# wenxuanliu/multimodal-vae

Measured on AMD Instinct MI355X. Metric: ELBO-steps/sec (whole node), MultiMNIST b=256 per GPU, higher is better.
Workload: dtype bf16; 1 GPU; multimnist_50x50_conv_mmvae_gru_text_3pass_elbo_step; batch_per_gpu=256, global_batch=256, n_latents=100, parallelism=dp1, hip_graph=False, optimizer=adam, mfma=bf16 in / fp32 acc; fp32 master weights, BN stats, PoE/KL/BCE/NLL, Adam

## Files before the change

### multimodal-vae_amd/csrc/convres.hip

```cpp
#include "gemm.h"
#include "convres_geo.h"
#include "convres.h"
#include "bn_dev.h"
#include "convres_epi.h"
#include <type_traits>
#include <cstdlib>

namespace {


template <int I, int N, typename F>
__device__ __forceinline__ void static_for(F&& f) {
    if constexpr (I < N) {
        f(std::integral_constant<int, I>{});
        static_for<I + 1, N>(f);
    }
}

struct ConvResArgs {
    const bf16* A;
    int nimg, group_n;
    const bf16* Wp[4];
    int Kpad[4];
    int Npad;
    bf16* out;
    int ldo;
    float2* colstats;
    const bf16* d_r;
    const float2* d_affine;
    const float2* d_meanrstd;
    float2* d_red;
    int dbg;
    BnFinalizeArgs fin;
    const bf16* t_r;
    const float2* t_red;
    const float2* t_mr;
    const float* t_gamma;
    float* t_dgamma; float* t_dbeta;
    float t_inv_cnt;
    int t_groups;
    bf16* stage_out;
    unsigned long long* ts;
};

constexpr unsigned OOB_OFF = 0x40000000u;

template <class G, int NI>
constexpr int tab_base(int c) {
    int r = 0;
    for (int i = 0; i < c; ++i) r += crgeo::cdiv(NI * G::OYX(i), 32) * 32;
    return r;
}

template <class G, int NI, int CH, int WAVES, int NG, bool SCR_OWN, int NSPLIT = 1, int KSPL = 1>
struct CrLayout {
    static constexpr int NTHR = WAVES * 64;
    static constexpr int MG = WAVES / (NG * KSPL), NT = G::N / 32 / NSPLIT / NG;
    static constexpr int max_mt() { int m = 0; for (int c = 0; c < G::NCLS; ++c) m = crgeo::cmax(m, crgeo::cdiv(crgeo::cdiv(NI * G::OYX(c), 32), MG)); return m; }
    static constexpr int RED_BYTES = KSPL > 1 ? WAVES * max_mt() * NT * 4096 : 0;
    static constexpr bool BDIR = CH == 0;
    static constexpr int BP = (CH * 16 + 8) * 2;
    static constexpr int W_BYTES = BDIR ? 0 : G::N * BP;
    static_assert(!BDIR || SCR_OWN, "direct-B kernels have no weight buffer to lend to the epilogue");
    static constexpr int IMG_ALL = NI * G::IMG_BYTES;
    static constexpr int TAB_BYTES = tab_base<G, NI>(G::NCLS) * 4;
    static constexpr int SCR_PITCH = 80, SCR_BYTES = 32 * SCR_PITCH;
    static constexpr int TRT_BYTES = G::C * 16;
    static constexpr int OFF_W = IMG_ALL, OFF_TAB = OFF_W + W_BYTES, OFF_TRT = OFF_TAB + TAB_BYTES,
                         OFF_SCR = OFF_TRT + TRT_BYTES, OFF_RED = OFF_SCR + (SCR_OWN ? WAVES * SCR_BYTES : 0), TOTAL = OFF_RED + RED_BYTES;
    static_assert((NSPLIT == 1 && KSPL == 1) || BDIR, "column / k splits exist for the direct-B kernels only");
    static_assert(G::N % (32 * NSPLIT * NG) == 0 && WAVES % (NG * KSPL) == 0, "wave decomposition");
    static_assert(SCR_OWN || W_BYTES >= WAVES * SCR_BYTES, "the weight buffer doubles as the epilogue scratch");
    static_assert(TOTAL <= 160 * 1024, "LDS budget");
};

template <class G, int NI, int CH, int WAVES, int NG, bool SCR_OWN, int MODE, int TR, int NSPLIT = 1, int KSPL = 1>
__global__ __launch_bounds__(WAVES * 64) void convres_kernel(const ConvResArgs a) {
    using L = CrLayout<G, NI, CH, WAVES, NG, SCR_OWN, NSPLIT, KSPL>;
    constexpr int NT = L::NT, MG = L::MG, NTHR = WAVES * 64;
    constexpr int BP = L::BP, SCR_PITCH = L::SCR_PITCH;
    extern __shared__ __attribute__((aligned(16))) char smem[];
    char* const img_s = smem;
    char* const w_s = smem + L::OFF_W;
    unsigned* const tab = reinterpret_cast<unsigned*>(smem + L::OFF_TAB);
    float4* const trt = reinterpret_cast<float4*>(smem + L::OFF_TRT);

    const int tid = threadIdx.x, lane = tid & 63;
    const int wave = __builtin_amdgcn_readfirstlane(tid >> 6);
    const int r = lane & 31, h = lane >> 5;
    const int kg = wave % KSPL, ng = (wave / KSPL) % NG, mg = wave / (KSPL * NG);
    const int ntb = blockIdx.y * (G::N / 32 / NSPLIT) + ng * NT;
    const int img0 = blockIdx.x * NI;
    const int grp = img0 / a.group_n;
    auto stamp = [&](int idx) {
        if (a.ts && lane == 0) a.ts[((size_t)blockIdx.x * WAVES + wave) * 16 + idx] = __builtin_amdgcn_s_memrealtime();
    };
    stamp(0);

    constexpr bool BDIR = L::BDIR;
    constexpr int WV = BDIR ? 1 : crgeo::cdiv(G::N * CH * 2, NTHR);
    i32x4c wreg[WV];
    auto w_fetch = [&](auto ci, auto chi) {
        constexpr int c = decltype(ci)::value, ch = decltype(chi)::value;
        constexpr int CHK = crgeo::cmin(CH, G::KSTEPS(c) - ch * CH), VPR = CHK * 2 + (BDIR ? 1 : 0), NV = G::N * VPR;
        const bf16* wsrc = a.Wp[c] + ch * CH * 16;
        const int kpad = a.Kpad[c];
#pragma unroll
        for (int it = 0; it < crgeo::cdiv(NV, NTHR); ++it) {
            const int v = tid + it * NTHR;
            const int n = v / VPR, kv = v - n * VPR;
            if (v < NV) wreg[it] = *reinterpret_cast<const i32x4c*>(wsrc + (size_t)n * kpad + kv * 8);
        }
    };
    auto w_store = [&](auto ci, auto chi) {
        constexpr int c = decltype(ci)::value, ch = decltype(chi)::value;
        constexpr int CHK = crgeo::cmin(CH, G::KSTEPS(c) - ch * CH), VPR = CHK * 2 + (BDIR ? 1 : 0), NV = G::N * VPR;
#pragma unroll
        for (int it = 0; it < crgeo::cdiv(NV, NTHR); ++it) {
            const int v = tid + it * NTHR;
            const int n = v / VPR, kv = v - n * VPR;
            if (v < NV) *reinterpret_cast<i32x4c*>(w_s + n * BP + kv * 16) = wreg[it];
        }
    };
    if constexpr (!BDIR) w_fetch(std::integral_constant<int, 0>{}, std::integral_constant<int, 0>{});

    constexpr int VPP = G::C / 8;
    constexpr int NVI = NI * G::AH * G::AW * VPP;
    constexpr int IT = crgeo::cdiv(NVI, NTHR), SB = 4, NB = crgeo::cdiv(IT, SB);
    static_assert(NTHR % VPP == 0, "a thread keeps its channel vector across staging iterations");
    const bf16* const src = a.A + (size_t)img0 * (G::AH * G::AW * G::C);
    const bf16* const src_r = TR == 2 ? a.t_r + (size_t)img0 * (G::AH * G::AW * G::C) : nullptr;
    bf16* const stage_dst = (TR != 0 && a.stage_out && blockIdx.y == 0) ? a.stage_out + (size_t)img0 * (G::AH * G::AW * G::C) : nullptr;
    i32x4c ireg[SB], rreg[TR == 2 ? SB : 1];
    auto i_fetch = [&](int b) {
#pragma unroll
        for (int i = 0; i < SB; ++i) {
            const int v = tid + (b * SB + i) * NTHR;
            if (b * SB + i < IT && v < NVI) {
                ireg[i] = *reinterpret_cast<const i32x4c*>(src + (size_t)v * 8);
                if constexpr (TR == 2) rreg[i] = *reinterpret_cast<const i32x4c*>(src_r + (size_t)v * 8);
            }
        }
    };
    float tc0[TR ? 8 : 1], tc1[TR ? 8 : 1], tc2[TR == 2 ? 8 : 1];
    auto i_store = [&](int b) {
#pragma unroll
        for (int i = 0; i < SB; ++i) {
            const int v = tid + (b * SB + i) * NTHR;
            if (b * SB + i < IT && v < NVI) {
                const int pix = v / VPP, cv = v - pix * VPP;
                const int img = pix / (G::AH * G::AW), p2 = pix - img * (G::AH * G::AW);
                const int iy = p2 / G::AW, ix = p2 - iy * G::AW;
                const int cell = G::cell(iy, ix);
                i32x4c val = ireg[i];
                if constexpr (TR == 1) {
                    const bf16x8 x = __builtin_bit_cast(bf16x8, val);
                    bf16x8 o;
#pragma unroll
                    for (int j = 0; j < 8; ++j) o[j] = (bf16)swish_fast((float)x[j] * tc0[j] + tc1[j]);
                    val = __builtin_bit_cast(i32x4c, o);
                } else if constexpr (TR == 2) {
                    const bf16x8 x = __builtin_bit_cast(bf16x8, val), rr = __builtin_bit_cast(bf16x8, rreg[i]);
                    bf16x8 o;
#pragma unroll
                    for (int j = 0; j < 8; ++j) o[j] = (bf16)((float)x[j] * tc0[j] + ((float)rr[j] * tc1[j] + tc2[j]));
                    val = __builtin_bit_cast(i32x4c, o);
                }
                if (cell >= 0) *reinterpret_cast<i32x4c*>(img_s + img * G::IMG_BYTES + cell + cv * 16) = val;
                if constexpr (TR != 0)
                    if (stage_dst) *reinterpret_cast<i32x4c*>(stage_dst + (size_t)v * 8) = val;
            }
        }
    };
    if (!(a.dbg & 4)) i_fetch(0);

    {
        const i32x4c z = {0, 0, 0, 0};
        for (int i = tid * 16; i < L::IMG_ALL; i += NTHR * 16) *reinterpret_cast<i32x4c*>(img_s + i) = z;
        const unsigned img_out = (unsigned)(G::OH * G::OW) * (unsigned)a.ldo * 2u;
        static_for<0, G::NCLS>([&](auto ci) {
            constexpr int c = decltype(ci)::value;
            constexpr int ROWS = NI * G::OYX(c), T = crgeo::cdiv(ROWS, 32);
            for (int e = tid; e < T * 32; e += NTHR) {
                unsigned v = OOB_OFF;
                if (e < ROWS) {
                    const int img = e / G::OYX(c), q = e - img * G::OYX(c);
                    const int jy = q / G::OX(c), jx = q - jy * G::OX(c);
                    v = (unsigned)img * img_out + (unsigned)((G::out_y(c, jy) * G::OW + G::out_x(c, jx)) * a.ldo * 2);
                }
                tab[tab_base<G, NI>(c) + e] = v;
            }
        });
        if constexpr (TR == 1) {
            for (int ch = tid; ch < G::C; ch += NTHR) {
                float2 aff, mr;
                bn_channel_tables(a.fin, grp, ch, aff, mr);
                trt[ch] = make_float4(aff.x, aff.y, 0.f, 0.f);
            }
            if (blockIdx.x == 0 && blockIdx.y == 0) {
                for (int i = tid; i < a.fin.G * G::C; i += NTHR) {
                    float2 aff, mr;
                    bn_channel_tables(a.fin, i / G::C, i % G::C, aff, mr);
                    a.fin.affine[i] = aff; a.fin.meanrstd[i] = mr;
                }
                bn_running_update(a.fin, tid, NTHR);
            }
        } else if constexpr (TR == 2) {
            for (int ch = tid; ch < G::C; ch += NTHR) {
                float sx = 0.f, sy = 0.f;
                for (int q = 0; q < MMVAE_STAT_SLOTS; ++q) {
                    const float2 t = a.t_red[((size_t)grp * MMVAE_STAT_SLOTS + q) * G::C + ch];
                    sx += t.x; sy += t.y;
                }
                const float2 mr = a.t_mr[grp * G::C + ch];
                const float g = a.t_gamma[ch] * mr.y, m1 = sx * a.t_inv_cnt, m2 = sy * a.t_inv_cnt;
                const float cb = -g * m2 * mr.y;
                trt[ch] = make_float4(g, cb, -cb * mr.x - g * m1, 0.f);
            }
            if (blockIdx.x == 0 && blockIdx.y == 0 && (a.t_dgamma || a.t_dbeta)) {
                for (int ch = tid; ch < G::C; ch += NTHR) {
                    float tg = 0.f, tb = 0.f;
                    for (int gg = 0; gg < a.t_groups; ++gg)
                        for (int q = 0; q < MMVAE_STAT_SLOTS; ++q) {
                            const float2 t = a.t_red[((size_t)gg * MMVAE_STAT_SLOTS + q) * G::C + ch];
                            tb += t.x; tg += t.y;
                        }
                    if (a.t_dgamma) a.t_dgamma[ch] += tg;
                    if (a.t_dbeta) a.t_dbeta[ch] += tb;
                }
            }
        }
    }
    stamp(1);
    __syncthreads();
    stamp(2);
    if constexpr (TR != 0) {
        const int cv0 = (tid % VPP) * 8;
#pragma unroll
        for (int j = 0; j < 8; ++j) {
            const float4 t = trt[cv0 + j];
            tc0[j] = t.x; tc1[j] = t.y;
            if constexpr (TR == 2) tc2[j] = t.z;
        }
    }
    if (!(a.dbg & 4)) {
        i_store(0);
        for (int b = 1; b < NB; ++b) { i_fetch(b); i_store(b); }
    }
    if constexpr (!BDIR) w_store(std::integral_constant<int, 0>{}, std::integral_constant<int, 0>{});
    stamp(3);
    __syncthreads();
    stamp(4);

    const __amdgpu_buffer_rsrc_t orsrc = __builtin_amdgcn_make_buffer_rsrc(
        a.out, 0, (int)((size_t)a.nimg * G::OH * G::OW * a.ldo * 2), 0x00020000);
    const __amdgpu_buffer_rsrc_t rrsrc = __builtin_amdgcn_make_buffer_rsrc(
        const_cast<bf16*>(a.d_r ? a.d_r : a.out), 0, (int)((size_t)a.nimg * G::OH * G::OW * a.ldo * 2), 0x00020000);
    const unsigned wg_out = (unsigned)img0 * (unsigned)(G::OH * G::OW) * (unsigned)a.ldo * 2u;
    float dsc[NT], dsh[NT], dmean[NT], drstd[NT], s1[NT], s2[NT];
#pragma unroll
    for (int nt = 0; nt < NT; ++nt) {
        const int co = (ntb + nt) * 32 + r;
        dsc[nt] = 1.f; dsh[nt] = 0.f; dmean[nt] = 0.f; drstd[nt] = 0.f; s1[nt] = 0.f; s2[nt] = 0.f;
        if (MODE == 1 && a.d_affine) { const float2 t = a.d_affine[grp * G::N + co]; dsc[nt] = t.x; dsh[nt] = t.y; }
        if (MODE == 1 && a.d_meanrstd) { const float2 t = a.d_meanrstd[grp * G::N + co]; dmean[nt] = t.x; drstd[nt] = t.y; }
    }
    char* const scr = (SCR_OWN ? smem + L::OFF_SCR : w_s) + wave * L::SCR_BYTES;
    __amdgpu_buffer_rsrc_t wrsrc[BDIR ? G::NCLS : 1];
    if constexpr (BDIR) {
#pragma unroll
        for (int i = 0; i < G::NCLS; ++i)
            wrsrc[i] = __builtin_amdgcn_make_buffer_rsrc(const_cast<bf16*>(a.Wp[i]), 0, a.Npad * a.Kpad[i] * 2, 0x00020000);
    }

    static_for<0, G::NCLS>([&](auto ci) {
        constexpr int c = decltype(ci)::value;
        constexpr int ROWS = NI * G::OYX(c), T = crgeo::cdiv(ROWS, 32), MT = crgeo::cdiv(T, MG);
        constexpr int KS = G::KSTEPS(c), CHE = BDIR ? KS : CH, NCH = crgeo::cdiv(KS, CHE);
        constexpr int KSL = KS / KSPL;
        int abase[MT];
#pragma unroll
        for (int m = 0; m < MT; ++m) {
            const int t = mg + m * MG;
            int R = (t < T ? t : 0) * 32 + r;
            R = R < ROWS ? R : ROWS - 1;
            const int img = R / G::OYX(c), q = R - img * G::OYX(c);
            const int jy = q / G::OX(c), jx = q - jy * G::OX(c);
            abase[m] = img * G::IMG_BYTES + G::base0(c) + jy * G::row_stride(c) + jx * G::col_stride(c) + h * 16;
            if constexpr (KSPL > 1) {
                static_assert(G::TH(c) % KSPL == 0, "the k split is by tap row");
                constexpr int KSL_ = KS / KSPL;
                abase[m] += kg * (G::step_off(c, KSL_) - G::step_off(c, 0));
            }
        }
        f32x16 acc[MT][NT];
#pragma unroll
        for (int m = 0; m < MT; ++m)
#pragma unroll
            for (int nt = 0; nt < NT; ++nt)
#pragma unroll
                for (int j = 0; j < 16; ++j) acc[m][nt][j] = 0.f;
        const int wrow = ((ng * NT) * 32 + r) * BP + h * 16;

        if constexpr (BDIR) {
            constexpr int PD = KSL < 8 ? KSL : 8;
            static_assert(KSPL == 1 || KSL % 2 == 0, "a wave's k range starts on a 32-column block of the packed weights");
            unsigned voff[NT];
#pragma unroll
            for (int nt = 0; nt < NT; ++nt)
                voff[nt] = (unsigned)(((2 * (ntb + nt) + (r >> 4)) * (a.Kpad[c] >> 5) * 64 + h * 16 + (r & 15)) * 16) +
                           (unsigned)(kg * (KSL / 2) * 1024);
            auto bload = [&](auto ki, bf16x8 (&fb)[NT]) {
                constexpr int kk = decltype(ki)::value;
#pragma unroll
                for (int nt = 0; nt < NT; ++nt)
                    fb[nt] = __builtin_bit_cast(bf16x8, __builtin_amdgcn_raw_buffer_load_b128(wrsrc[c], (int)voff[nt], (kk >> 1) * 1024 + (kk & 1) * 512, 0));
            };
            auto aload = [&](auto ki, bf16x8 (&fa)[MT]) {
                constexpr int kk = decltype(ki)::value;
                constexpr int aoff = G::step_off(c, kk);
#pragma unroll
                for (int m = 0; m < MT; ++m) fa[m] = *reinterpret_cast<const bf16x8*>(img_s + abase[m] + aoff);
            };
            bf16x8 bq[PD][NT], af[MT];
            static_for<0, PD>([&](auto pi) { bload(pi, bq[decltype(pi)::value]); });
            aload(std::integral_constant<int, 0>{}, af);
            __builtin_amdgcn_sched_group_barrier(0x100, MT, 0);
            if (!(a.dbg & 2))
            static_for<0, KSL>([&](auto ki) {
                constexpr int kk = decltype(ki)::value;
                constexpr int KS = KSL;
                bf16x8 bcur[NT], an[MT];
#pragma unroll
                for (int nt = 0; nt < NT; ++nt) bcur[nt] = bq[kk % PD][nt];
                if constexpr (kk + PD < KS) bload(std::integral_constant<int, kk + PD>{}, bq[kk % PD]);
                if constexpr (kk + 1 < KS) aload(std::integral_constant<int, kk + 1>{}, an);
#pragma unroll
                for (int m = 0; m < MT; ++m)
#pragma unroll
                    for (int nt = 0; nt < NT; ++nt)
                        acc[m][nt] = __builtin_amdgcn_mfma_f32_32x32x16_bf16(af[m], bcur[nt], acc[m][nt], 0, 0, 0);
                if constexpr (kk + PD < KS) __builtin_amdgcn_sched_group_barrier(0x020, NT, 0);
                if constexpr (kk + 1 < KS) __builtin_amdgcn_sched_group_barrier(0x100, MT, 0);
                __builtin_amdgcn_sched_group_barrier(0x008, MT * NT, 0);
                if constexpr (kk + 1 < KS) {
#pragma unroll
                    for (int m = 0; m < MT; ++m) af[m] = an[m];
                }
            });
            if constexpr (KSPL > 1) {
                float* const red = reinterpret_cast<float*>(smem + L::OFF_RED);
                constexpr int WSTR = L::max_mt() * NT * 1024;
#pragma unroll
                for (int m = 0; m < MT; ++m)
#pragma unroll
                    for (int nt = 0; nt < NT; ++nt)
#pragma unroll
                        for (int v4 = 0; v4 < 4; ++v4)
                            *reinterpret_cast<f32x4*>(red + wave * WSTR + ((m * NT + nt) * 64 + lane) * 16 + v4 * 4) =
                                f32x4{acc[m][nt][4 * v4], acc[m][nt][4 * v4 + 1], acc[m][nt][4 * v4 + 2], acc[m][nt][4 * v4 + 3]};
                __syncthreads();
                if (kg == 0) {
#pragma unroll
                    for (int k2 = 1; k2 < KSPL; ++k2)
#pragma unroll
                        for (int m = 0; m < MT; ++m)
#pragma unroll
                            for (int nt = 0; nt < NT; ++nt)
#pragma unroll
                                for (int v4 = 0; v4 < 4; ++v4) {
                                    const f32x4 t = *reinterpret_cast<const f32x4*>(red + (wave + k2) * WSTR + ((m * NT + nt) * 64 + lane) * 16 + v4 * 4);
                                    acc[m][nt][4 * v4] += t[0]; acc[m][nt][4 * v4 + 1] += t[1];
                                    acc[m][nt][4 * v4 + 2] += t[2]; acc[m][nt][4 * v4 + 3] += t[3];
                                }
                }
                __syncthreads();
            }
        }
        static_for<0, NCH>([&](auto chi) {
            constexpr int ch = decltype(chi)::value;
            constexpr int CHK = crgeo::cmin(CHE, KS - ch * CHE);
            constexpr bool last_chunk = ch + 1 == NCH;
            constexpr bool has_next = !BDIR && (!last_chunk || c + 1 < G::NCLS);
            constexpr int cn = last_chunk ? c + 1 : c, chn = last_chunk ? 0 : ch + 1;
            if constexpr (has_next) w_fetch(std::integral_constant<int, cn>{}, std::integral_constant<int, chn>{});
            if (!BDIR && !(a.dbg & 2)) {
                bf16x8 af[MT], bfr[NT];
                auto frag = [&](auto ki, bf16x8 (&fa)[MT], bf16x8 (&fb)[NT]) {
                    constexpr int kk = decltype(ki)::value;
                    constexpr int aoff = G::step_off(c, ch * CHE + kk);
#pragma unroll
                    for (int nt = 0; nt < NT; ++nt)
                        fb[nt] = *reinterpret_cast<const bf16x8*>(w_s + wrow + nt * 32 * BP + kk * 32);
#pragma unroll
                    for (int m = 0; m < MT; ++m) fa[m] = *reinterpret_cast<const bf16x8*>(img_s + abase[m] + aoff);
                };
                frag(std::integral_constant<int, 0>{}, af, bfr);
                __builtin_amdgcn_sched_group_barrier(0x100, MT + NT, 0);
                static_for<0, CHK>([&](auto ki) {
                    constexpr int kk = decltype(ki)::value;
                    bf16x8 an[MT], bn[NT];
                    if constexpr (kk + 1 < CHK) frag(std::integral_constant<int, kk + 1>{}, an, bn);
#pragma unroll
                    for (int m = 0; m < MT; ++m)
#pragma unroll
                        for (int nt = 0; nt < NT; ++nt)
                            acc[m][nt] = __builtin_amdgcn_mfma_f32_32x32x16_bf16(af[m], bfr[nt], acc[m][nt], 0, 0, 0);
                    if constexpr (kk + 1 < CHK) __builtin_amdgcn_sched_group_barrier(0x100, MT + NT, 0);
                    __builtin_amdgcn_sched_group_barrier(0x008, MT * NT, 0);
                    if constexpr (kk + 1 < CHK) {
#pragma unroll
                        for (int m = 0; m < MT; ++m) af[m] = an[m];
#pragma unroll
                        for (int nt = 0; nt < NT; ++nt) bfr[nt] = bn[nt];
                    }
                });
            }
            if constexpr (last_chunk) {
                stamp(5 + 2 * c);
                if constexpr (!SCR_OWN) __syncthreads();
#pragma unroll
                for (int m = 0; m < MT; ++m) {
                    const int t = mg + m * MG;
                    if (t < T && kg == 0) {
                        const unsigned* trow = tab + tab_base<G, NI>(c) + t * 32;
                        const unsigned off0 = trow[lane & 15], off1 = trow[16 + (lane & 15)];
                        const int rows_left = ROWS - t * 32;
#pragma unroll
                        for (int nt = 0; nt < NT; ++nt) {
                            const unsigned cob = (unsigned)(((ntb + nt) * 32 + (lane >> 4) * 8) * 2) + wg_out;
                            if (rows_left >= 32)
                                cr_epilogue_tile<MODE, false>(acc[m][nt], scr, lane, 32, off0 + cob, off1 + cob, orsrc, rrsrc,
                                                              dsc[nt], dsh[nt], dmean[nt], drstd[nt], s1[nt], s2[nt], !(a.dbg & 1));
                            else
                                cr_epilogue_tile<MODE, true>(acc[m][nt], scr, lane, rows_left, off0 + cob, off1 + cob, orsrc, rrsrc,
                                                             dsc[nt], dsh[nt], dmean[nt], drstd[nt], s1[nt], s2[nt], !(a.dbg & 1));
                        }
                    }
                }
            }
            if constexpr (last_chunk) stamp(6 + 2 * c);
            if constexpr (has_next) {
                __syncthreads();
                w_store(std::integral_constant<int, cn>{}, std::integral_constant<int, chn>{});
                __syncthreads();
            }
        });
    });

    stamp(13);
    float2* red = MODE == 1 ? a.d_red : a.colstats;
    if (red && kg == 0) {
        const int slot = (int)(blockIdx.x + wave) % MMVAE_STAT_SLOTS;
#pragma unroll
        for (int nt = 0; nt < NT; ++nt) {
            const float t1 = s1[nt] + __shfl_xor(s1[nt], 32, 64), t2 = s2[nt] + __shfl_xor(s2[nt], 32, 64);
            if (h == 0) {
                float2* d = red + ((size_t)grp * MMVAE_STAT_SLOTS + slot) * G::N + (ntb + nt) * 32 + r;
                atomicAdd(&d->x, t1);
                atomicAdd(&d->y, t2);
            }
        }
    }
    stamp(14);
}

}

namespace {

template <class G>
bool geo_matches(const GemmParams& p) {
    const GatherCommon& c = p.c;
    if (c.C != G::C || c.Ald != G::C || c.N != G::N || c.AH != G::AH || c.AW != G::AW || c.OH != G::OH || c.OW != G::OW) return false;
    if (c.nclasses != G::NCLS) return false;
    if (G::FORM == 0) {
        if (c.sy != G::S || c.sx != G::S || c.dy != 1 || c.dx != 1 || c.osy != 1 || c.osx != 1) return false;
    } else {
        if (c.sy != 1 || c.sx != 1 || c.dy != -1 || c.dx != -1 || c.osy != G::S || c.osx != G::S) return false;
    }
    for (int i = 0; i < G::NCLS; ++i) {
        const GatherClass& k = p.cls[i];
        if (k.OY != G::OY(i) || k.OX != G::OX(i) || k.TH != G::TH(i) || k.TW != G::TW(i) || k.offy != G::offy(i) ||
            k.offx != G::offx(i) || k.ooy != G::ph(i) || k.oox != G::pw(i) || k.K != G::K(i) || k.Kpad < G::K(i))
            return false;
    }
    return true;
}

template <class G, int NI, int CH, int WAVES, int NG, bool SCR_OWN, int MODE, int TR, int NSPLIT, int KSPL>
int launch_cr_mode(const ConvResArgs& a, hipStream_t stream) {
    using L = CrLayout<G, NI, CH, WAVES, NG, SCR_OWN, NSPLIT, KSPL>;
    static std::atomic<unsigned> attr_set{0};
    if (mmvae_first_use_on_device(attr_set))
        hipFuncSetAttribute(reinterpret_cast<const void*>(&convres_kernel<G, NI, CH, WAVES, NG, SCR_OWN, MODE, TR, NSPLIT, KSPL>),
                            hipFuncAttributeMaxDynamicSharedMemorySize, 160 * 1024);
    MMVAE_LAUNCH((convres_kernel<G, NI, CH, WAVES, NG, SCR_OWN, MODE, TR, NSPLIT, KSPL>), dim3(a.nimg / NI, NSPLIT), dim3(WAVES * 64), L::TOTAL, stream, a);
    MMVAE_TRY(mmvae_check_launch("convres"));
    return 1;
}

template <class G, int NI, int CH, int WAVES, int NG, bool SCR_OWN, int NSPLIT = 1, int KSPL = 1>
int launch_cr(const GemmParams& p, hipStream_t stream) {
    const GatherCommon& c = p.c;
    const int nimg = c.groups * c.group_n;
    ConvResArgs a{};
    a.A = c.A; a.nimg = nimg; a.group_n = c.group_n;
    constexpr bool BDIR = CH == 0;
    for (int i = 0; i < G::NCLS; ++i) {
        a.Wp[i] = BDIR ? p.cls[i].Wf : p.cls[i].Wp; a.Kpad[i] = p.cls[i].Kpad;
        if (BDIR && (!a.Wp[i] || a.Kpad[i] % 32 != 0)) return 0;
    }
    a.Npad = p.npad;
    a.out = p.out_bf; a.ldo = p.ldo; a.colstats = p.colstats;
    a.dbg = mmvae_knob("convres_dbg", 0);
    a.ts = reinterpret_cast<unsigned long long*>(((unsigned long long)(unsigned)mmvae_knob("convres_ts_hi", 0) << 32) |
                                                 (unsigned)mmvae_knob("convres_ts_lo", 0));
    a.d_r = p.d_r; a.d_affine = p.d_affine; a.d_meanrstd = p.d_meanrstd; a.d_red = p.d_red;
    const int kind = p.tr ? p.tr->kind : 0;
    MMVAE_REQUIRE(!(p.tr && p.tr->out == c.A) || NSPLIT == 1, "convres: an in-place staging by-product needs one workgroup per image tile");
    if (mmvae_probe_on()) {
        char tag[96];
        snprintf(tag, sizeof(tag), "convres form%d %d>%d %dx%d>%dx%d k%d s%d %s tr%d img%d", G::FORM, G::C, G::N, G::AH, G::AW, G::OH, G::OW,
                 G::KH, G::S, p.d_r ? "dgrad" : "fwd", kind, nimg);
        mmvae_probe_tag(tag, 2.0 * (G::FORM == 0 ? G::OH * G::OW : G::AH * G::AW) * G::KH * G::KW * G::C * G::N * (double)nimg);
    }
    if (kind == 1) {
        a.fin = p.tr->fin; a.stage_out = p.tr->out;
        MMVAE_REQUIRE(a.fin.C == G::C && a.fin.G == c.groups && a.fin.affine && a.fin.meanrstd && a.fin.gamma && a.fin.beta,
                      "convres: BatchNorm tables of the staged operand do not match the layer");
        MMVAE_REQUIRE(!p.d_r, "convres: forward-type staging transform on a data-gradient launch");
        return launch_cr_mode<G, NI, CH, WAVES, NG, SCR_OWN, 0, 1, NSPLIT, KSPL>(a, stream);
    }
    if (kind == 2) {
        const GatherTransform& t = *p.tr;
        MMVAE_REQUIRE(p.d_r && t.r && t.red && t.mr && t.gamma && t.groups == c.groups, "convres: BatchNorm-backward staging needs r / sums / tables");
        a.t_r = t.r; a.t_red = t.red; a.t_mr = t.mr; a.t_gamma = t.gamma; a.t_dgamma = t.dgamma; a.t_dbeta = t.dbeta;
        a.t_inv_cnt = t.inv_cnt; a.t_groups = t.groups; a.stage_out = t.out;
        return launch_cr_mode<G, NI, CH, WAVES, NG, SCR_OWN, 1, 2, NSPLIT, KSPL>(a, stream);
    }
    return p.d_r ? launch_cr_mode<G, NI, CH, WAVES, NG, SCR_OWN, 1, 0, NSPLIT, KSPL>(a, stream)
                 : launch_cr_mode<G, NI, CH, WAVES, NG, SCR_OWN, 0, 0, NSPLIT, KSPL>(a, stream);
}

bool features_ok(const GemmParams& p) {
    const GatherCommon& c = p.c;
    if (!p.out_bf || p.out_f || p.out_act_bf || p.e_mask || p.d_mask || p.d_colsum || p.d_cmod > 0 || p.d_bcast_n > 0) return false;
    if (c.a_bcast_n > 0 || c.a_mask || c.a_affine || c.a_act != ACT_NONE) return false;
    if (p.ldo != c.N || p.bias) return false;
    if (p.d_r && (p.d_ld != p.ldo || p.d_act != ACT_SWISH)) return false;
    if (p.colstats && p.d_r) return false;
    if ((size_t)c.groups * c.group_n * c.OH * c.OW * p.ldo * 2 >= (size_t)OOB_OFF) return false;
    return true;
}

template <class G, int NI, int CH, int WAVES, int NG, bool SCR_OWN, int NSPLIT = 1, int KSPL = 1>
int try_cr(const GemmParams& p, hipStream_t stream) {
    if (!geo_matches<G>(p)) return 0;
    if (p.c.group_n % NI != 0) return 0;
    return launch_cr<G, NI, CH, WAVES, NG, SCR_OWN, NSPLIT, KSPL>(p, stream);
}

using crgeo::Geo;
typedef Geo<0, 32, 64, 25, 25, 12, 12, 4, 4, 2, 1> G_mm_conv2;
typedef Geo<0, 64, 128, 12, 12, 6, 6, 4, 4, 2, 1> G_mm_conv3;
typedef Geo<1, 128, 64, 6, 6, 12, 12, 4, 4, 2, 1> G_mm_convT2;
typedef Geo<1, 64, 32, 12, 12, 25, 25, 5, 5, 2, 1> G_mm_convT3;
typedef Geo<1, 64, 32, 12, 12, 25, 25, 4, 4, 2, 1> G_mm_conv2d;
typedef Geo<0, 32, 64, 25, 25, 12, 12, 5, 5, 2, 1> G_mm_convT3d;
typedef Geo<1, 256, 128, 2, 2, 6, 6, 4, 4, 2, 0> G_mm_convT1;
typedef Geo<0, 128, 256, 6, 6, 2, 2, 4, 4, 2, 0> G_mm_conv4;
typedef Geo<0, 32, 64, 32, 32, 16, 16, 4, 4, 2, 1> G_ca_conv2;
typedef Geo<0, 64, 128, 16, 16, 8, 8, 4, 4, 2, 1> G_ca_conv3;
typedef Geo<1, 128, 64, 8, 8, 16, 16, 4, 4, 2, 1> G_ca_convT2;
typedef Geo<1, 64, 32, 16, 16, 32, 32, 4, 4, 2, 1> G_ca_convT3;

}

int try_launch_convres(const GemmParams& p, hipStream_t stream) {
    const bool forced = p.tr && p.tr->kind != 0;
    if ((!mmvae_knob("convres", 1) && !forced) || !features_ok(p)) {
        MMVAE_REQUIRE(!forced, "convres: a staging transform was requested for a launch this path does not cover");
        return 0;
    }
    int rc;
    const int nimg = p.c.groups * p.c.group_n;
    const int alt = mmvae_knob("convres_alt", 0);
    if ((rc = try_cr<G_mm_conv2, 1, 16, 8, 2, true>(p, stream)) != 0) return rc;
    if (alt != 3) {
        if ((rc = try_cr<G_mm_conv3, 2, 0, 8, 4, true>(p, stream)) != 0) return rc;
        if (nimg <= 256) { if ((rc = try_cr<G_mm_convT2, 2, 0, 8, 2, true>(p, stream)) != 0) return rc; }
        if ((rc = try_cr<G_mm_convT2, 4, 0, 8, 2, true>(p, stream)) != 0) return rc;
    }
    if ((rc = try_cr<G_mm_conv3, 2, 8, 8, 4, true>(p, stream)) != 0) return rc;
    if (nimg <= 256) { if ((rc = try_cr<G_mm_convT2, 2, 8, 4, 1, true>(p, stream)) != 0) return rc; }
    if ((rc = try_cr<G_mm_convT2, 4, 16, 8, 2, true>(p, stream)) != 0) return rc;
    if (alt == 1) { if ((rc = try_cr<G_mm_convT3, 4, 20, 8, 1, false>(p, stream)) != 0) return rc; }
    if ((rc = try_cr<G_mm_convT3, 2, 16, 4, 1, false>(p, stream)) != 0) return rc;
    if ((rc = try_cr<G_mm_conv2d, 1, 16, 8, 1, true>(p, stream)) != 0) return rc;
    if (alt != 4) {
        if (nimg > 256 && alt != 5) { if ((rc = try_cr<G_mm_convT1, 16, 0, 5, 1, true, 4, 1>(p, stream)) != 0) return rc; }
        if ((rc = try_cr<G_mm_convT1, 8, 0, 6, 1, true, 4, 2>(p, stream)) != 0) return rc;
        if ((rc = try_cr<G_mm_conv4, 8, 0, 8, 2, true, 4, 4>(p, stream)) != 0) return rc;
    }
    if ((rc = try_cr<G_mm_convT3d, 2, 10, 8, 2, false>(p, stream)) != 0) return rc;
    if (mmvae_knob("convres_celeba", 1)) {
        if ((rc = try_cr<G_ca_conv2, 1, 16, 8, 2, true>(p, stream)) != 0) return rc;
        if ((rc = try_cr<G_ca_conv3, 2, 0, 8, 4, true>(p, stream)) != 0) return rc;
        if ((rc = try_cr<G_ca_convT2, 4, 0, 8, 2, true>(p, stream)) != 0) return rc;
        if ((rc = try_cr<G_ca_convT3, 2, 16, 4, 1, false>(p, stream)) != 0) return rc;
    }
    MMVAE_REQUIRE(!forced, "convres: no kernel is compiled for the geometry of a launch with a staging transform");
    return 0;
}
```

### multimodal-vae_amd/csrc/convres_geo.h

```cpp
#pragma once

namespace crgeo {

constexpr int cdiv(int a, int b) { return (a + b - 1) / b; }
constexpr int fdiv(int a, int b) { return a >= 0 ? a / b : -((-a + b - 1) / b); }
constexpr int cmax(int a, int b) { return a > b ? a : b; }
constexpr int cmin(int a, int b) { return a < b ? a : b; }

template <int FORM_, int C_, int N_, int AH_, int AW_, int OH_, int OW_, int KH_, int KW_, int S_, int PAD_, int PIXPAD_ = 16>
struct Geo {
    static constexpr int FORM = FORM_, C = C_, N = N_, AH = AH_, AW = AW_, OH = OH_, OW = OW_, KH = KH_, KW = KW_, S = S_, PAD = PAD_;
    static constexpr int NCLS = FORM == 0 ? 1 : S * S;
    static constexpr int PIX = C * 2 + PIXPAD_;
    static constexpr int KSTEP_PER_TAP = C / 16;
    static_assert(C % 8 == 0 && N % 32 == 0, "channel counts");

    static constexpr int ph(int c) { return FORM == 0 ? 0 : c / S; }
    static constexpr int pw(int c) { return FORM == 0 ? 0 : c % S; }
    static constexpr int kh0(int c) { return (ph(c) + PAD) % S; }
    static constexpr int kw0(int c) { return (pw(c) + PAD) % S; }
    static constexpr int OY(int c) { return FORM == 0 ? OH : (OH - ph(c) + S - 1) / S; }
    static constexpr int OX(int c) { return FORM == 0 ? OW : (OW - pw(c) + S - 1) / S; }
    static constexpr int TH(int c) { return FORM == 0 ? KH : (KH - kh0(c) + S - 1) / S; }
    static constexpr int TW(int c) { return FORM == 0 ? KW : (KW - kw0(c) + S - 1) / S; }
    static constexpr int offy(int c) { return FORM == 0 ? -PAD : (ph(c) + PAD - kh0(c)) / S; }
    static constexpr int offx(int c) { return FORM == 0 ? -PAD : (pw(c) + PAD - kw0(c)) / S; }
    static constexpr int K(int c) { return TH(c) * TW(c) * C; }
    static constexpr int KSTEPS(int c) { return K(c) / 16; }
    static constexpr int OYX(int c) { return OY(c) * OX(c); }
    static constexpr int TPI(int c) { return cdiv(OYX(c), 32); }
    static constexpr int osy() { return FORM == 0 ? 1 : S; }
    static constexpr int out_y(int c, int jy) { return jy * osy() + ph(c); }
    static constexpr int out_x(int c, int jx) { return jx * osy() + pw(c); }
    static constexpr int gy(int c, int jy, int ty) { return FORM == 0 ? jy * S - PAD + ty : jy + offy(c) - ty; }
    static constexpr int gx(int c, int jx, int tx) { return FORM == 0 ? jx * S - PAD + tx : jx + offx(c) - tx; }

    static constexpr int DMIN = fdiv(-PAD, S), DMAX = fdiv(KW - 1 - PAD, S);
    static constexpr int PW0 = OW + DMAX - DMIN;
    static constexpr int LR0 = (OH - 1) * S + KH;
    static constexpr int ring_lo(bool x) {
        int r = 0;
        for (int c = 0; c < NCLS; ++c) r = cmax(r, x ? TW(c) - 1 - offx(c) : TH(c) - 1 - offy(c));
        return r;
    }
    static constexpr int ring_hi(bool x) {
        int r = 0;
        for (int c = 0; c < NCLS; ++c) r = cmax(r, x ? OX(c) - 1 + offx(c) - (AW - 1) : OY(c) - 1 + offy(c) - (AH - 1));
        return r;
    }
    static constexpr int RT = FORM == 1 ? ring_lo(false) : 0, RB = FORM == 1 ? ring_hi(false) : 0;
    static constexpr int RL = FORM == 1 ? ring_lo(true) : 0, RR = FORM == 1 ? ring_hi(true) : 0;
    static constexpr int AHP = RT + AH + RB, AWP = RL + AW + RR;
    static constexpr int IMG_BYTES = FORM == 0 ? LR0 * S * PW0 * PIX : AHP * AWP * PIX;

    static constexpr int cell(int iy, int ix) {
        if (FORM == 0) {
            const int row = iy + PAD, plane = ix % S, col = ix / S - DMIN;
            if (row < 0 || row >= LR0 || col < 0 || col >= PW0) return -1;
            return ((row * S + plane) * PW0 + col) * PIX;
        }
        return ((iy + RT) * AWP + ix + RL) * PIX;
    }
    static constexpr int row_stride(int) { return FORM == 0 ? S * S * PW0 * PIX : AWP * PIX; }
    static constexpr int col_stride(int) { return PIX; }
    static constexpr int base0(int c) {
        return FORM == 0 ? 0 : ((offy(c) + RT - (TH(c) - 1)) * AWP + offx(c) + RL - (TW(c) - 1)) * PIX;
    }
    static constexpr int tap_off(int c, int ty, int tx) {
        if (FORM == 0) {
            const int e = tx - PAD, d = fdiv(e, S), p = e - d * S;
            return ((ty * S + p) * PW0 + d - DMIN) * PIX;
        }
        return ((TH(c) - 1 - ty) * AWP + (TW(c) - 1 - tx)) * PIX;
    }
    static constexpr int step_tap(int kk) { return kk / KSTEP_PER_TAP; }
    static constexpr int step_c0(int kk) { return (kk % KSTEP_PER_TAP) * 16; }
    static constexpr int step_off(int c, int kk) {
        const int tap = step_tap(kk);
        return tap_off(c, tap / TW(c), tap % TW(c)) + step_c0(kk) * 2;
    }
    static constexpr int max_ksteps() { int r = 0; for (int c = 0; c < NCLS; ++c) r = cmax(r, KSTEPS(c)); return r; }
    static constexpr int max_tpi() { int r = 0; for (int c = 0; c < NCLS; ++c) r = cmax(r, TPI(c)); return r; }
    static constexpr int tab_entries() { int r = 0; for (int c = 0; c < NCLS; ++c) r += TPI(c) * 32; return r; }
    static constexpr int tab_base(int c) { int r = 0; for (int i = 0; i < c; ++i) r += TPI(i) * 32; return r; }
};

}
```

### multimodal-vae_amd/csrc/gemm.h

```cpp
#pragma once
#include "common.h"
#include "elementwise.h"
#include <vector>

#define MMVAE_MAX_CLASSES 4

struct GatherClass {
    int OY, OX;
    int rows_per_group;
    int TH, TW;
    int offy, offx;
    int ooy, oox;
    int K;
    int Kpad;
    const bf16* Wp;
    const bf16* Wf;
    float* dWp;
};

struct GatherCommon {
    int groups, group_n;
    const bf16* A;
    int AH, AW, Ald, C;
    int sy, sx, dy, dx;
    const float2* a_affine;
    int a_act;
    const uint8_t* a_mask;
    float a_mask_scale;
    int a_bcast_n;
    int OH, OW, osy, osx;
    int N;
    int nclasses;
};

struct GatherTransform {
    int kind;
    BnFinalizeArgs fin;
    const bf16* r;
    const float2* red;
    const float2* mr;
    const float* gamma;
    float* dgamma; float* dbeta;
    float inv_cnt;
    int groups;
    bf16* out;
};

struct GemmParams {
    GatherCommon c;
    GatherClass cls[MMVAE_MAX_CLASSES];
    int ksplit;
    float* sk_buf;
    unsigned* sk_cnt;
    const float* bias;
    bf16* out_bf;
    float* out_f;
    int ldo;
    bf16* out_act_bf;
    int e_act;
    const uint8_t* e_mask;
    float e_mask_scale;
    float2* colstats;
    const bf16* d_r;
    int d_ld;
    int d_bcast_n;
    const float2* d_affine;
    int d_act;
    const uint8_t* d_mask;
    float d_mask_scale;
    const float2* d_meanrstd;
    float2* d_red;
    float* d_colsum;
    int npad;
    const GatherTransform* tr;
    int d_cmod;
};

struct WgradParams {
    GatherCommon c;
    GatherClass cls[MMVAE_MAX_CLASSES];
    const bf16* P;
    int ldp;
    const float2* p_affine;
    int p_act;
    int rows_per_block;
    float* slab;
    long long slab_chunk_stride;
    long long slab_cls_off[MMVAE_MAX_CLASSES];
};

struct WgradSlabJob { float* dst; const float* slab; int N, K, Kpad, chunks; long long chunk_stride; hipStream_t stream;
                      int src_ld; };
struct WgradRingJob { float* dst; const float* slab; int N, Kpad, C, Kc, copies, ntx, ty0, tx0, st, kw; hipStream_t stream; };
struct WgradSlabCtx {
    float* pool = nullptr;
    size_t cap = 0, used = 0;
    std::vector<WgradSlabJob> jobs;
    std::vector<WgradRingJob> ring_jobs;
    void reset(float* p, size_t c) { pool = p; cap = c; used = 0; jobs.clear(); ring_jobs.clear(); }
    float* take(size_t n) {
        n = (n + 3) / 4 * 4;
        if (!pool || used + n > cap) return nullptr;
        float* p = pool + used;
        used += n;
        return p;
    }
};

int launch_gemm_gather(const GemmParams& p, hipStream_t stream);
int try_launch_gemm_small(const GemmParams& p, hipStream_t stream);
int launch_wgrad(const WgradParams& p, hipStream_t stream, WgradSlabCtx* ctx = nullptr);
int launch_wgrad_group(const WgradParams* list, int n, hipStream_t stream, WgradSlabCtx* ctx = nullptr);
int launch_wgrad_reduce(WgradSlabCtx* ctx, hipStream_t stream, bool only_own = false);
```

### multimodal-vae_amd/csrc/multimnist.hip

```cpp
#include "multimnist.h"
#include <memory>
#include "mlp_tail.h"
#include "plan_base.h"
#include "thin.h"
#include <cstring>

namespace {
constexpr int IMG = 50, NPIX = 2500;
}

struct MMPlan : PlanBase {
    int ldz, kx, kz;
    ConvL conv[4], convT[4];
    LinL fc[3], up;
    BnL bn[6];
    struct GruIdx { int wih, whh, wihT, whhT, g_wih, g_whh; long long bih, bhh; } te_f, te_r, td0, td1;
    const float* step_image = nullptr;
    hipEvent_t ev_dz = nullptr;
    hipEvent_t ev_txtgrads = nullptr;
    int te_h2p, te_h2pT, g_te_h2p, td_z2h, td_z2hT, g_td_z2h, td_h2o, td_h2oT, g_td_h2o;
    bool mlp_tail = false;
    int mt_w2, mt_w3, mt_w3t, mt_w2t;
    struct W {
        char* zero_begin; size_t zero_bytes;
        float2 *st_e[3], *red_e[3], *st_d[3], *red_d[3];
        float* sums; float* dz_img; float* dz_txt;
        float2 *aff_e[3], *mr_e[3], *aff_d[3], *mr_d[3];
        bf16 *patches1, *r1, *r2, *r3, *r4, *y1, *y2;
        bf16 *a1, *a2, *a3, *a4, *ay1, *ay2, *au, *aq1, *aq2, *aq3;
        float* encout; uint8_t *m1, *m2, *gkeep;
        float *txtout, *te_gates_f, *te_gates_r; bf16 *te_x, *te_hprev, *te_hsum;
        float *eps, *mu, *logvar, *z_f32; bf16* z_bf;
        bf16 *u, *q1, *q2, *q3; float *logits, *recon, *dlogit;
        float *words, *dwords, *td_gates; long long* tokens;
        bf16 *td_x0, *td_h0p, *td_mid, *td_h1p, *td_hz, *td_zbf;
        bf16 *dgi0, *dgh0, *dgi1, *dgh1, *dlogit_bf, *dhinit;
        bf16 *patches4, *d3, *d2, *d1, *du;
        bf16 *d_encout; float* d_txtout; bf16* te_dout_bf; bf16 *te_dgi_f, *te_dgh_f, *te_dgi_r;
        bf16 *dy2, *dy1, *db4, *dr4, *d3e, *d2e, *d1e;
        bf16 *d3r, *d2r, *d1r, *d3er, *d2er;
        float* tmp_f32;
        float* slab; size_t slab_floats;
    } w;
};

namespace {

void build_params(MMPlan& P) {
    const int D = P.D;
    auto bn = [&](const std::string& n, int c) { add_param(P, n + ".weight", {c}); add_param(P, n + ".bias", {c}); };
    auto gru = [&](const std::string& n, int inp, const char* sfx) {
        add_param(P, n + ".weight_ih_" + sfx, {300, inp}); add_param(P, n + ".weight_hh_" + sfx, {300, 100});
        add_param(P, n + ".bias_ih_" + sfx, {300}); add_param(P, n + ".bias_hh_" + sfx, {300});
    };
    add_param(P, "image_encoder.features.0.weight", {32, 1, 4, 4});
    add_param(P, "image_encoder.features.2.weight", {64, 32, 4, 4}); bn("image_encoder.features.3", 64);
    add_param(P, "image_encoder.features.5.weight", {128, 64, 4, 4}); bn("image_encoder.features.6", 128);
    add_param(P, "image_encoder.features.8.weight", {256, 128, 4, 4}); bn("image_encoder.features.9", 256);
    add_param(P, "image_encoder.classifier.0.weight", {400, 1024}); add_param(P, "image_encoder.classifier.0.bias", {400});
    add_param(P, "image_encoder.classifier.3.weight", {200, 400}); add_param(P, "image_encoder.classifier.3.bias", {200});
    add_param(P, "image_encoder.classifier.6.weight", {2 * D, 200}); add_param(P, "image_encoder.classifier.6.bias", {2 * D});
    add_param(P, "image_decoder.upsample.0.weight", {1024, D}); add_param(P, "image_decoder.upsample.0.bias", {1024});
    add_param(P, "image_decoder.hallucinate.0.weight", {256, 128, 4, 4}); bn("image_decoder.hallucinate.1", 128);
    add_param(P, "image_decoder.hallucinate.3.weight", {128, 64, 4, 4}); bn("image_decoder.hallucinate.4", 64);
    add_param(P, "image_decoder.hallucinate.6.weight", {64, 32, 5, 5}); bn("image_decoder.hallucinate.7", 32);
    add_param(P, "image_decoder.hallucinate.9.weight", {32, 1, 4, 4});
    add_param(P, "text_encoder.embed.weight", {12, 100});
    gru("text_encoder.gru", 100, "l0"); gru("text_encoder.gru", 100, "l0_reverse");
    add_param(P, "text_encoder.h2p.weight", {2 * D, 100}); add_param(P, "text_encoder.h2p.bias", {2 * D});
    add_param(P, "text_decoder.embed.weight", {12, 100});
    add_param(P, "text_decoder.z2h.weight", {100, D}); add_param(P, "text_decoder.z2h.bias", {100});
    gru("text_decoder.gru", 100 + D, "l0"); gru("text_decoder.gru", 100, "l1");
    add_param(P, "text_decoder.h2o.weight", {12, 100 + D}); add_param(P, "text_decoder.h2o.bias", {12});
}

void build_plan(MMPlan& P) {
    const int D = P.D;
    P.ldz = round_up(D + 1, 8); P.kz = round_up(D, 32); P.kx = round_up(100 + D, 32);
    build_params(P);
    const char* bnn[6] = {"image_encoder.features.3", "image_encoder.features.6", "image_encoder.features.9",
                          "image_decoder.hallucinate.1", "image_decoder.hallucinate.4", "image_decoder.hallucinate.7"};
    const int bnc[6] = {64, 128, 256, 128, 64, 32};
    long long so = 0;
    for (int i = 0; i < 6; ++i) {
        P.bn[i] = BnL{off(P, std::string(bnn[i]) + ".weight"), off(P, std::string(bnn[i]) + ".bias"), bnc[i], so, i};
        P.bn_names.push_back(bnn[i]); P.bn_list.push_back(P.bn[i]);
        so += 2 * bnc[i];
    }
    build_conv(P, P.conv[0], "image_encoder.features.0.weight", ConvGeom{1, 32, 4, 4, 2, 1, 50, 50, 25, 25, false}, -1, false, true, false);
    build_conv(P, P.conv[1], "image_encoder.features.2.weight", ConvGeom{32, 64, 4, 4, 2, 1, 25, 25, 12, 12, false}, 0, true, false, false);
    build_conv(P, P.conv[2], "image_encoder.features.5.weight", ConvGeom{64, 128, 4, 4, 2, 1, 12, 12, 6, 6, false}, 1, true, false, false);
    build_conv(P, P.conv[3], "image_encoder.features.8.weight", ConvGeom{128, 256, 4, 4, 2, 0, 6, 6, 2, 2, false}, 2, true, false, false);
    build_conv(P, P.convT[0], "image_decoder.hallucinate.0.weight", ConvGeom{256, 128, 4, 4, 2, 0, 2, 2, 6, 6, true}, 3, true, false, false);
    build_conv(P, P.convT[1], "image_decoder.hallucinate.3.weight", ConvGeom{128, 64, 4, 4, 2, 1, 6, 6, 12, 12, true}, 4, true, false, false);
    build_conv(P, P.convT[2], "image_decoder.hallucinate.6.weight", ConvGeom{64, 32, 5, 5, 2, 1, 12, 12, 25, 25, true}, 5, true, false, false);
    build_conv(P, P.convT[3], "image_decoder.hallucinate.9.weight", ConvGeom{32, 1, 4, 4, 2, 1, 25, 25, 50, 50, true}, -1, true, false, true);
    add_frag_packs(P, P.conv[2]);
    add_frag_packs(P, P.convT[1]);
    add_frag_packs(P, P.conv[3]);
    add_frag_packs(P, P.convT[0]);

    {
        LinL& f = P.fc[0];
        f.w_off = off(P, "image_encoder.classifier.0.weight"); f.b_off = off(P, "image_encoder.classifier.0.bias");
        f.N = 400; f.K = 1024; f.pk_dgrad = -1;
        PackDesc d = pack_dense(f.w_off, 400, 1024, npad_for(400), 1024, 1024, 0);
        d.TW = 2; d.C = 256; d.s_ty = 2; d.s_tx = 1; d.s_c = 4;
        f.pk_fwd = P.pk.add(d);
        PackDesc gd = d; gd.Npad = round_up(400, 64);
        f.gk = P.gk.add(gd);
        for (int sidx = 0; sidx < 4; ++sidx)
            f.pk_dgrad4[sidx] = P.pk.add(pack_dense(f.w_off + sidx, 256, 400, npad_for(256), round_up(400, 64), 4, 1024));
    }
    auto lin = [&](LinL& f, const std::string& n, int N, int K) {
        f.w_off = off(P, n + ".weight"); f.b_off = off(P, n + ".bias"); f.N = N; f.K = K;
        f.pk_fwd = P.pk.add(pack_dense(f.w_off, N, K, npad_for(N), round_up(round_up(K, 8), 64), K, 1));
        f.gk = P.gk.add(pack_dense(f.w_off, N, K, round_up(N, 64), round_up(round_up(K, 8), 64), K, 1));
        f.pk_dgrad = P.pk.add(pack_dense(f.w_off, K, N, npad_for(K), round_up(round_up(N, 8), 64), 1, K));
    };
    lin(P.fc[1], "image_encoder.classifier.3", 200, 400);
    lin(P.fc[2], "image_encoder.classifier.6", 2 * D, 200);
    if (D == 100) {
        P.mlp_tail = true;
        auto fragd = [&](PackDesc d) { d.frag = 1; return P.pk.add(d); };
        P.mt_w2 = fragd(pack_dense(P.fc[1].w_off, 200, 400, 208, 416, 400, 1));
        P.mt_w3 = fragd(pack_dense(P.fc[2].w_off, 200, 200, 208, 224, 200, 1));
        P.mt_w3t = fragd(pack_dense(P.fc[2].w_off, 200, 200, 208, 224, 1, 200));
        P.mt_w2t = fragd(pack_dense(P.fc[1].w_off, 400, 200, 400, 224, 1, 400));
    }
    {
        LinL& f = P.up;
        f.w_off = off(P, "image_decoder.upsample.0.weight"); f.b_off = off(P, "image_decoder.upsample.0.bias");
        f.N = 1024; f.K = D;
        PackDesc d = pack_dense(f.w_off, 1024, D, npad_for(1024), round_up(P.ldz, 64), 0, 1);
        d.NL = 256; d.s_nhi = D; d.s_nlo = 4 * D;
        d.bias_off = f.b_off; d.b_nhi = 1; d.b_nlo = 4;
        f.pk_fwd = P.pk.add(d);
        PackDesc gd = d; f.gk = P.gk.add(gd);
        PackDesc t = pack_dense(f.w_off, D, 1024, npad_for(D), 1024, 1, 0);
        t.TW = 4; t.C = 256; t.s_ty = 0; t.s_tx = D; t.s_c = 4 * D;
        f.pk_dgrad = P.pk.add(t);
    }
    auto rt = [&](long long w, int N, int K, bool transpose) {
        PackDesc d = transpose ? pack_dense(w, K, N, round_up(K, 16), round_up(N, 32), 1, K) : pack_dense(w, N, K, round_up(N, 16), round_up(K, 32), K, 1);
        d.frag = 1;
        return P.pk.add(d);
    };
    auto gw = [&](long long w, int N, int K, int Kc) {
        return P.gk.add(pack_dense(w, N, K, round_up(N, 64), round_up(Kc, 64), K, 1));
    };
    auto grui = [&](MMPlan::GruIdx& g, const std::string& n, const char* sfx, int inp, int inp_k, bool need_hh) {
        const long long wih = off(P, n + ".weight_ih_" + sfx), whh = off(P, n + ".weight_hh_" + sfx);
        g.bih = off(P, n + ".bias_ih_" + sfx); g.bhh = off(P, n + ".bias_hh_" + sfx);
        g.wih = rt(wih, 300, inp, false); g.wihT = rt(wih, 300, inp, true);
        g.whh = rt(whh, 300, 100, false); g.whhT = rt(whh, 300, 100, true);
        g.g_wih = gw(wih, 300, inp, inp_k);
        g.g_whh = need_hh ? gw(whh, 300, 100, TXT_HP) : -1;
    };
    grui(P.te_f, "text_encoder.gru", "l0", 100, TXT_HP, true);
    grui(P.te_r, "text_encoder.gru", "l0_reverse", 100, TXT_HP, false);
    {
        const long long w = off(P, "text_encoder.h2p.weight");
        P.te_h2p = rt(w, 2 * D, 100, false); P.te_h2pT = rt(w, 2 * D, 100, true); P.g_te_h2p = gw(w, 2 * D, 100, TXT_HP);
    }
    {
        const long long w = off(P, "text_decoder.z2h.weight");
        P.td_z2h = rt(w, 100, D, false); P.td_z2hT = rt(w, 100, D, true); P.g_td_z2h = gw(w, 100, D, P.kz);
    }
    grui(P.td0, "text_decoder.gru", "l0", 100 + D, P.kx, true);
    grui(P.td1, "text_decoder.gru", "l1", 100, TXT_HP, true);
    {
        const long long w = off(P, "text_decoder.h2o.weight");
        P.td_h2o = rt(w, 12, 100 + D, false); P.td_h2oT = rt(w, 12, 100 + D, true); P.g_td_h2o = gw(w, 12, 100 + D, P.kx);
    }
    for (PackDesc& d : P.pk.d) {
        d.part = 0;
        for (const ParamInfo& pi : P.params)
            if (d.src_off >= pi.offset && d.src_off < pi.offset + pi.numel)
                d.part = pi.name.rfind("text_", 0) == 0 ? 1 : pi.name.rfind("image_decoder.", 0) == 0 ? 2 : 0;
    }
    {
        auto late = [&](int idx) { if (idx >= 0) P.pk.d[idx].part = 2; };
        for (int l = 0; l < 4; ++l)
            for (int i = 0; i < 4; ++i) { late(P.conv[l].pk_dgrad[i]); late(P.conv[l].pk_dgrad_f[i]); }
        for (int i = 0; i < 4; ++i) late(P.fc[0].pk_dgrad4[i]);
        late(P.fc[1].pk_dgrad); late(P.fc[2].pk_dgrad);
        if (P.mlp_tail) { late(P.mt_w3t); late(P.mt_w2t); }
    }
    for (PackDesc& d : P.gk.d)
        for (const ParamInfo& pi : P.params)
            if (d.src_off >= pi.offset && d.src_off < pi.offset + pi.numel)
                d.part = pi.name.rfind("image_decoder.", 0) == 0 || pi.name.rfind("text_decoder.", 0) == 0;
}

void carve(MMPlan& P, Workspace& ws) {
    MMPlan::W& w = P.w;
    const size_t B = P.B, D = P.D, B3 = (size_t)P.carve_passes * B, B2 = (size_t)(P.carve_passes < 2 ? P.carve_passes : 2) * B;
    char* z0 = ws.take<char>(0);
    const int ec[3] = {64, 128, 256}, dc[3] = {128, 64, 32};
    const int SS = MMVAE_STAT_SLOTS;
    for (int i = 0; i < 3; ++i) { w.st_e[i] = ws.take<float2>(SS * ec[i]); w.red_e[i] = ws.take<float2>(SS * ec[i]); }
    for (int i = 0; i < 3; ++i) { w.st_d[i] = ws.take<float2>(3 * SS * dc[i]); w.red_d[i] = ws.take<float2>(3 * SS * dc[i]); }
    w.sums = ws.take<float>(16 * MMVAE_LOSS_SLOTS);
    P.sk_cnt = ws.take<unsigned>(1024);
    w.dz_img = ws.take<float>(B3 * D);
    w.dz_txt = ws.take<float>(B3 * D);
    char* z1 = ws.take<char>(0);
    w.zero_begin = z0; w.zero_bytes = (size_t)(z1 - z0);
    for (int i = 0; i < 3; ++i) { w.aff_e[i] = ws.take<float2>(ec[i]); w.mr_e[i] = ws.take<float2>(ec[i]); }
    for (int i = 0; i < 3; ++i) { w.aff_d[i] = ws.take<float2>(3 * dc[i]); w.mr_d[i] = ws.take<float2>(3 * dc[i]); }
    w.patches1 = ws.take<bf16>(B * 625 * 16);
    w.r1 = ws.take<bf16>(B * 625 * 32); w.r2 = ws.take<bf16>(B * 144 * 64); w.r3 = ws.take<bf16>(B * 36 * 128);
    w.r4 = ws.take<bf16>(B * 4 * 256);
    w.y1 = ws.take<bf16>(B2 * 400); w.y2 = ws.take<bf16>(B2 * 200);
    w.a1 = ws.take<bf16>(B * 625 * 32); w.a2 = ws.take<bf16>(B * 144 * 64); w.a3 = ws.take<bf16>(B * 36 * 128);
    w.a4 = ws.take<bf16>(B * 4 * 256); w.ay1 = ws.take<bf16>(B2 * 400); w.ay2 = ws.take<bf16>(B2 * 200);
    w.au = ws.take<bf16>(B3 * 1024); w.aq1 = ws.take<bf16>(B3 * 36 * 128); w.aq2 = ws.take<bf16>(B3 * 144 * 64);
    w.aq3 = ws.take<bf16>(B3 * 625 * 32);
    w.encout = ws.take<float>(B2 * 2 * D);
    w.m1 = ws.take<uint8_t>(B2 * 400); w.m2 = ws.take<uint8_t>(B2 * 200); w.gkeep = ws.take<uint8_t>(4 * B3 * 100);
    w.txtout = ws.take<float>(B * 2 * D);
    w.te_gates_f = ws.take<float>(4 * 5 * B * 100); w.te_gates_r = ws.take<float>(5 * B * 100);
    w.te_x = ws.take<bf16>(4 * B * 128); w.te_hprev = ws.take<bf16>(4 * B * 128); w.te_hsum = ws.take<bf16>(B * 128);
    w.eps = ws.take<float>(B3 * D); w.mu = ws.take<float>(B3 * D); w.logvar = ws.take<float>(B3 * D);
    w.z_f32 = ws.take<float>(B3 * D); w.z_bf = ws.take<bf16>(B3 * P.ldz);
    w.u = ws.take<bf16>(B3 * 1024); w.q1 = ws.take<bf16>(B3 * 36 * 128); w.q2 = ws.take<bf16>(B3 * 144 * 64);
    w.q3 = ws.take<bf16>(B3 * 625 * 32);
    w.logits = ws.take<float>(B3 * NPIX); w.recon = ws.take<float>(B3 * NPIX); w.dlogit = ws.take<float>(B3 * NPIX);
    w.words = ws.take<float>(B3 * 48); w.dwords = ws.take<float>(B3 * 48); w.tokens = ws.take<long long>(B3 * 4);
    w.td_gates = ws.take<float>(4 * 2 * 5 * B3 * 100);
    w.td_x0 = ws.take<bf16>(4 * B3 * P.kx); w.td_hz = ws.take<bf16>(4 * B3 * P.kx);
    w.td_h0p = ws.take<bf16>(4 * B3 * 128); w.td_mid = ws.take<bf16>(4 * B3 * 128); w.td_h1p = ws.take<bf16>(4 * B3 * 128);
    w.td_zbf = ws.take<bf16>(B3 * P.kz);
    w.dgi0 = ws.take<bf16>(4 * B3 * 304); w.dgh0 = ws.take<bf16>(4 * B3 * 304);
    w.dgi1 = ws.take<bf16>(4 * B3 * 304); w.dgh1 = ws.take<bf16>(4 * B3 * 304);
    w.dlogit_bf = ws.take<bf16>(4 * B3 * 16); w.dhinit = ws.take<bf16>(B3 * 112);
    w.patches4 = ws.take<bf16>(B3 * 625 * 16);
    w.d3 = ws.take<bf16>(B3 * 625 * 32); w.d2 = ws.take<bf16>(B3 * 144 * 64); w.d1 = ws.take<bf16>(B3 * 36 * 128);
    w.du = ws.take<bf16>(B3 * 1024);
    w.d_encout = ws.take<bf16>(B2 * 2 * D); w.d_txtout = ws.take<float>(B * 2 * D);
    w.te_dout_bf = ws.take<bf16>(B * round_up(2 * (int)D, 8));
    w.te_dgi_f = ws.take<bf16>(4 * B * 304); w.te_dgh_f = ws.take<bf16>(4 * B * 304); w.te_dgi_r = ws.take<bf16>(B * 304);
    w.dy2 = ws.take<bf16>(B2 * 200); w.dy1 = ws.take<bf16>(B2 * 400);
    w.db4 = ws.take<bf16>(B2 * 1024); w.dr4 = ws.take<bf16>(B * 1024);
    w.d3e = ws.take<bf16>(B * 36 * 128); w.d2e = ws.take<bf16>(B * 144 * 64); w.d1e = ws.take<bf16>(B * 625 * 32);
    w.d3r = ws.take<bf16>(B3 * 625 * 32); w.d2r = ws.take<bf16>(B3 * 144 * 64); w.d1r = ws.take<bf16>(B3 * 36 * 128);
    w.d3er = ws.take<bf16>(B * 36 * 128); w.d2er = ws.take<bf16>(B * 144 * 64);
    w.tmp_f32 = ws.take<float>(B3 * NPIX);
    P.sk_floats = (size_t)256 * 128 * 128;
    P.sk_buf = ws.take<float>(P.sk_floats);
    w.slab_floats = (size_t)(P.carve_passes >= 3 ? 48 : 16) << 20;
    w.slab = ws.take<float>(w.slab_floats);
}

int enc_fwd(MMPlan& P, const float* image, int variants, const uint8_t* m1, const uint8_t* m2, int dropout, int training,
            int bn_updates, float* out, hipStream_t s, bool fuse = false) {
    MMPlan::W& w = P.w;
    const int B = P.B;
    if (fuse && mmvae_knob("mm_conv1_mfma", 1)) {
        const PackDesc& d = P.pk.d[P.conv[0].pk_fwd[0]];
        MMVAE_TRY(launch_conv1_fwd_mfma(image, B, P.buf.packed + d.dst_off, d.Kpad, w.r1, w.a1, s));
    } else {
    MMVAE_TRY(launch_im2col_small(image, B, 1, IMG, IMG, 4, 4, 2, 1, 25, 25, w.patches1, 16, s));
    {
        GatherPlan pl = dense_plan(B * 625, 16, 16, 32);
        GemmParams g = gemm_of(P, pl, P.conv[0].pk_fwd, 1, B * 625);
        g.c.A = w.patches1; g.out_bf = w.r1; g.ldo = 32; g.out_act_bf = w.a1; g.e_act = ACT_SWISH;
        MMVAE_TRY(launch_gemm_gather(g, s));
    }
    }
    bf16* r[4] = {w.r1, w.r2, w.r3, w.r4};
    bf16* a[4] = {w.a1, w.a2, w.a3, w.a4};
    for (int l = 1; l < 4; ++l) {
        const ConvL& L = P.conv[l];
        GemmParams g = gemm_of(P, L.fwd, L.pk_fwd, 1, B, L.pk_fwd_f);
        g.c.A = a[l - 1];
        g.out_bf = r[l]; g.ldo = L.g.Cout;
        g.colstats = training ? w.st_e[l - 1] : nullptr;
        GatherTransform tr{};
        if (fuse && l >= 2) {
            const int prows = B * P.conv[l - 1].g.OH * P.conv[l - 1].g.OW;
            tr.kind = 1;
            tr.fin = bn_fin_args(P, P.bn[P.conv[l - 1].bn], prows, 1, w.st_e[l - 2], bn_updates, w.aff_e[l - 2], w.mr_e[l - 2], training);
            g.c.A = r[l - 1]; g.tr = &tr;
            if (mmvae_knob("mm_stage_out", 1)) tr.out = a[l - 1];
        }
        MMVAE_TRY(launch_gemm_gather(g, s));
        const int rows = B * L.g.OH * L.g.OW;
        if (fuse && l <= 2) continue;
        MMVAE_TRY(bn_act(P, P.bn[L.bn], r[l], a[l], rows, rows, 1, w.st_e[l - 1], bn_updates, w.aff_e[l - 1], w.mr_e[l - 1], training, s));
    }
    const int rows = variants * B;
    const bool drop = training && dropout;
    const float ms = 1.f / (1.f - DROP_P);
    {
        GatherPlan pl = plan_fwdform(2, 2, 1, 1, 256, 2, 2, 1, 0, 400, 1, rows);
        GemmParams g = gemm_of(P, pl, &P.fc[0].pk_fwd, 1, rows);
        g.c.A = w.a4; g.c.a_bcast_n = B;
        g.bias = P.buf.params + P.fc[0].b_off; g.out_bf = w.y1; g.ldo = 400;
        g.out_act_bf = w.ay1; g.e_act = ACT_SWISH; if (drop) { g.e_mask = m1; g.e_mask_scale = ms; }
        MMVAE_TRY(launch_gemm_gather(g, s));
    }
    if (P.mlp_tail) {
        Mlp2FwdArgs a{};
        a.rows = rows; a.x = w.ay1;
        a.w2 = P.buf.packed + P.pk.d[P.mt_w2].dst_off; a.b2 = P.buf.params + P.fc[1].b_off;
        a.w3 = P.buf.packed + P.pk.d[P.mt_w3].dst_off; a.b3 = P.buf.params + P.fc[2].b_off;
        if (drop) { a.mask = m2; a.mask_scale = ms; }
        a.y2 = w.y2; a.ay2 = w.ay2; a.out = out;
        return launch_mlp2_fwd(a, s);
    }
    {
        GatherPlan pl = dense_plan(rows, 400, 400, 200);
        GemmParams g = gemm_of(P, pl, &P.fc[1].pk_fwd, 1, rows);
        g.c.A = w.ay1;
        g.bias = P.buf.params + P.fc[1].b_off; g.out_bf = w.y2; g.ldo = 200;
        g.out_act_bf = w.ay2; g.e_act = ACT_SWISH; if (drop) { g.e_mask = m2; g.e_mask_scale = ms; }
        MMVAE_TRY(launch_gemm_gather(g, s));
    }
    {
        GatherPlan pl = dense_plan(rows, 200, 200, 2 * P.D);
        GemmParams g = gemm_of(P, pl, &P.fc[2].pk_fwd, 1, rows);
        g.c.A = w.ay2;
        g.bias = P.buf.params + P.fc[2].b_off; g.out_f = out; g.ldo = 2 * P.D;
        MMVAE_TRY(launch_gemm_gather(g, s));
    }
    return MMVAE_OK;
}

int enc_bwd(MMPlan& P, const bf16* d_out, int variants, const uint8_t* m1, const uint8_t* m2, int dropout, hipStream_t s, bool fuse = false) {
    MMPlan::W& w = P.w;
    const int B = P.B, rows = variants * B, D2 = 2 * P.D;
    const float ms = 1.f / (1.f - DROP_P);
    auto cls_w = std::make_shared<std::vector<WgradParams>>();
    if (P.mlp_tail) {
        {
            GatherPlan pl = dense_plan(rows, 200, 200, D2);
            WgradParams g = wgrad_of(P, pl, &P.fc[2].gk, 1, rows);
            g.c.A = w.ay2; g.P = d_out; g.ldp = D2;
            if (fuse) cls_w->push_back(g);
            else MMVAE_TRY(wgrad_async(P, g, s));
        }
        Mlp2BwdArgs a{};
        a.rows = rows; a.d_out = d_out;
        a.w3t = P.buf.packed + P.pk.d[P.mt_w3t].dst_off; a.w2t = P.buf.packed + P.pk.d[P.mt_w2t].dst_off;
        a.y2 = w.y2; a.y1 = w.y1;
        if (dropout) { a.mask2 = m2; a.mask1 = m1; a.mask_scale = ms; }
        a.dy2 = w.dy2; a.dy1 = w.dy1;
        a.db2 = P.buf.grads + P.fc[1].b_off; a.db1 = P.buf.grads + P.fc[0].b_off;
        MMVAE_TRY(launch_mlp2_bwd(a, s));
        GatherPlan pl = dense_plan(rows, 400, 400, 200);
        WgradParams g = wgrad_of(P, pl, &P.fc[1].gk, 1, rows);
        g.c.A = w.ay1; g.P = w.dy2; g.ldp = 200;
        if (fuse) cls_w->push_back(g);
        else MMVAE_TRY(wgrad_async(P, g, s));
    } else {
    {
        GatherPlan pl = dense_plan(rows, 200, 200, D2);
        WgradParams g = wgrad_of(P, pl, &P.fc[2].gk, 1, rows);
        g.c.A = w.ay2; g.P = d_out; g.ldp = D2;
        MMVAE_TRY(wgrad_async(P, g, s));
        GatherPlan pd = dense_plan(rows, D2, D2, 200);
        GemmParams d = gemm_of(P, pd, &P.fc[2].pk_dgrad, 1, rows);
        d.c.A = d_out; d.out_bf = w.dy2; d.ldo = 200;
        d.d_r = w.y2; d.d_ld = 200; d.d_act = ACT_SWISH; if (dropout) { d.d_mask = m2; d.d_mask_scale = ms; }
        d.d_colsum = P.buf.grads + P.fc[1].b_off;
        MMVAE_TRY(launch_gemm_gather(d, s));
    }
    {
        GatherPlan pl = dense_plan(rows, 400, 400, 200);
        WgradParams g = wgrad_of(P, pl, &P.fc[1].gk, 1, rows);
        g.c.A = w.ay1; g.P = w.dy2; g.ldp = 200;
        MMVAE_TRY(wgrad_async(P, g, s));
        GatherPlan pd = dense_plan(rows, 200, 200, 400);
        GemmParams d = gemm_of(P, pd, &P.fc[1].pk_dgrad, 1, rows);
        d.c.A = w.dy2; d.out_bf = w.dy1; d.ldo = 400;
        d.d_r = w.y1; d.d_ld = 400; d.d_act = ACT_SWISH; if (dropout) { d.d_mask = m1; d.d_mask_scale = ms; }
        d.d_colsum = P.buf.grads + P.fc[0].b_off;
        MMVAE_TRY(launch_gemm_gather(d, s));
    }
    }
    {
        GatherPlan pl = plan_fwdform(2, 2, 1, 1, 256, 2, 2, 1, 0, 400, 1, rows);
        WgradParams g = wgrad_of(P, pl, &P.fc[0].gk, 1, rows);
        g.c.A = w.a4; g.c.a_bcast_n = B;
        g.P = w.dy1; g.ldp = 400;
        if (P.mlp_tail && fuse) {
            MMPlan* pp = &P;
            cls_w->push_back(g);
            side_later(P, [pp, cls_w](hipStream_t ws_) {
                MMVAE_TRY(launch_wgrad_group(cls_w->data(), (int)cls_w->size(), ws_, &pp->slab));
                return pp->batch_reduce ? MMVAE_OK : launch_wgrad_reduce(&pp->slab, ws_, true);
            }, mmvae_knob("mm_cls_lane", 1));
        } else {
            MMVAE_TRY(wgrad_async(P, g, s));
        }
        GatherPlan pd{};
        pd.c.AH = 1; pd.c.AW = 1; pd.c.Ald = 400; pd.c.C = 400; pd.c.sy = pd.c.sx = 1; pd.c.dy = pd.c.dx = 1;
        pd.c.OH = 2; pd.c.OW = 2; pd.c.osy = pd.c.osx = 1; pd.c.N = 256; pd.c.nclasses = 4;
        for (int sidx = 0; sidx < 4; ++sidx) {
            GatherClass& k = pd.cls[sidx];
            k.OY = 1; k.OX = 1; k.TH = 1; k.TW = 1; k.offy = 0; k.offx = 0; k.ooy = sidx / 2; k.oox = sidx % 2;
            k.K = 400; k.Kpad = round_up(400, 64);
        }
        GemmParams d = gemm_of(P, pd, P.fc[0].pk_dgrad4, 1, rows);
        d.c.A = w.dy1; d.out_bf = w.db4; d.ldo = 256;
        d.d_r = w.r4; d.d_ld = 256; d.d_bcast_n = B; d.d_act = ACT_SWISH;
        d.d_affine = w.aff_e[2]; d.d_meanrstd = w.mr_e[2]; d.d_red = w.red_e[2];
        MMVAE_TRY(launch_gemm_gather(d, s));
    }
    bf16* r[4] = {w.r1, w.r2, w.r3, w.r4};
    bf16* a[4] = {w.a1, w.a2, w.a3, w.a4};
    bf16* dr[4] = {w.d1e, w.d2e, w.d3e, w.dr4};
    bf16* drr[4] = {nullptr, w.d2er, w.d3er, nullptr};
    for (int l = 3; l >= 1; --l) {
        const ConvL& L = P.conv[l];
        const BnL& b = P.bn[L.bn];
        const int pix = L.g.OH * L.g.OW;
        const bool fl = fuse && l < 3;
        BnBwdApplyArgs x{};
        x.db = (l == 3) ? w.db4 : dr[l];
        x.db2 = (l == 3 && variants == 2) ? w.db4 + (size_t)B * 1024 : nullptr;
        x.r = r[l]; x.dr = fl ? drr[l] : dr[l]; x.rows = B * pix; x.C = L.g.Cout; x.ld = L.g.Cout; x.rows_per_group = B * pix; x.G = 1;
        x.red = w.red_e[l - 1]; x.meanrstd = w.mr_e[l - 1]; x.gamma = P.buf.params + b.w_off;
        x.dgamma = P.buf.grads + b.w_off; x.dbeta = P.buf.grads + b.b_off;
        if (!fl) MMVAE_TRY(launch_bn_bwd_apply(x, s));
        WgradParams gw = wgrad_of(P, L.fwd, L.gk, 1, B);
        gw.c.A = a[l - 1]; gw.P = x.dr; gw.ldp = L.g.Cout;
        if (fuse) {
            MMPlan* pp = &P;
            {
                const bool byp = mmvae_knob("mm_stage_out", 1) != 0;
                const bool actp = l >= 2 && !byp;
                const bool bnb = fl && !(byp && l == 2);
                const int prows = B * P.conv[l >= 2 ? l - 1 : 1].g.OH * P.conv[l >= 2 ? l - 1 : 1].g.OW;
                const BnL bp = P.bn[P.conv[l >= 2 ? l - 1 : 1].bn];
                const bf16* rin = r[l >= 2 ? l - 1 : 1]; bf16* ao = a[l >= 2 ? l - 1 : 1]; const float2* st = w.st_e[l >= 2 ? l - 2 : 0];
                WgradParams g0 = wgrad_of(P, L.fwd, L.gk, 1, B);
                g0.c.A = a[l - 1]; g0.P = x.dr; g0.ldp = L.g.Cout;
                side_later(P, [pp, x, g0, bnb, actp, bp, rin, ao, st, prows](hipStream_t ws_) {
                    if (bnb) MMVAE_TRY(launch_bn_bwd_apply(x, ws_));
                    if (actp) MMVAE_TRY(bn_act_side(*pp, bp, rin, ao, prows, prows, 1, st, 1, ws_));
                    return wgrad_on(*pp, g0, ws_);
                }, l == 1 ? 1 : l == 2 ? mmvae_knob("mm_conv3_lane", 0) : mmvae_knob("mm_conv4_lane", 0));
            }
            if (fuse && l == 1) MMVAE_TRY(side_flush(P, s));
        }
        {
            GemmParams d = gemm_of(P, L.dgrad, L.pk_dgrad, 1, B, L.pk_dgrad_f);
            d.c.A = dr[l]; d.out_bf = dr[l - 1]; d.ldo = L.g.Cin;
            d.d_r = r[l - 1]; d.d_ld = L.g.Cin; d.d_act = ACT_SWISH;
            if (l > 1) { d.d_affine = w.aff_e[l - 2]; d.d_meanrstd = w.mr_e[l - 2]; d.d_red = w.red_e[l - 2]; }
            GatherTransform tr{};
            if (fl) {
                tr.kind = 2; tr.r = r[l]; tr.red = w.red_e[l - 1]; tr.mr = w.mr_e[l - 1]; tr.gamma = P.buf.params + b.w_off;
                tr.inv_cnt = 1.f / (float)(B * pix); tr.groups = 1;
                if (l == 2 && mmvae_knob("mm_stage_out", 1)) {
                    tr.out = drr[l]; tr.dgamma = P.buf.grads + b.w_off; tr.dbeta = P.buf.grads + b.b_off;
                }
                d.tr = &tr;
            }
            const bool flush = fuse && P.wgrad_forked && (mmvae_knob("mm_forks", 0) ? l == 2 : l >= 2);
            if (flush) arm_fork(P);
            MMVAE_TRY(launch_gemm_gather(d, s));
            if (flush) { MMVAE_TRY(commit_fork(P, s)); MMVAE_TRY(side_flush(P, s)); }
        }
        if (!fuse) MMVAE_TRY(wgrad_async(P, gw, s));
    }
    if (fuse && !P.wgrad_forked) MMVAE_TRY(side_flush(P, s));
    if (fuse && mmvae_knob("mm_conv1_mfma", 1) && P.step_image) {
        const PackDesc& gd = P.gk.d[P.conv[0].gk[0]];
        MMVAE_TRY(launch_conv1_wgrad_mfma(P.step_image, B, w.d1e, P.buf.gpk + gd.dst_off, gd.Kpad, s));
    } else {
        GatherPlan pl = dense_plan(B * 625, 16, 16, 32);
        WgradParams g = wgrad_of(P, pl, P.conv[0].gk, 1, B * 625);
        g.c.A = w.patches1; g.P = w.d1e; g.ldp = 32;
        MMVAE_TRY(launch_wgrad(g, s, nullptr));
    }
    return MMVAE_OK;
}

int fused_tail(MMPlan& P, int groups, int training, const ConvTLastFwdArgs* last, int last_groups, int fused_bwd_groups, hipStream_t s) {
    MMPlan::W& w = P.w;
    const int B = P.B;
    const ConvL& L = P.convT[2];
    const BnL& b = P.bn[L.bn];
    DecLastFusedArgs x{};
    x.r = w.q3; x.act = ACT_SWISH; x.w = P.buf.params + P.convT[3].w_off;
    x.G = last_groups > 0 ? last_groups : groups; x.B = B; x.IH = 25; x.IW = 25; x.Cin = 32;
    x.bwd_groups = std::min(fused_bwd_groups, x.G);
    BnFinalizeArgs& f = x.fin;
    f.stats = w.st_d[2]; f.G = groups; f.C = b.C; f.count = (float)(B * L.g.OH * L.g.OW);
    f.gamma = P.buf.params + b.w_off; f.beta = P.buf.params + b.b_off;
    f.running_mean = P.buf.bn_stats + b.stat_off; f.running_var = P.buf.bn_stats + b.stat_off + b.C;
    f.num_batches_tracked = P.buf.bn_nbt + b.idx;
    f.updates_per_group = 1; f.affine = w.aff_d[2]; f.meanrstd = w.mr_d[2]; f.eps = BN_EPS; f.momentum = BN_MOM; f.training = training;
    f.skip_update_mask = groups > 1 ? P.dec_skip_mask : 0u;
    x.target = last->target; x.logits = last->logits; x.recon = last->recon; x.dlogit = nullptr;
    for (int k = 0; k < 4; ++k) x.coef[k] = last->coef[k];
    x.loss_sum = last->loss_sum;
    if (last->loglik) { x.loglik = last->loglik; x.rows_per_target = last->rows_per_target; x.B = last->rows; }
    if (x.bwd_groups > 0) {
        const int chunks = x.bwd_groups * B * (dec_last_mfma_applies(x) ? 1 : dec_last_fused_strips(25));
        x.wslab = P.slab.take((size_t)chunks * 32 * 16);
        MMVAE_REQUIRE(x.wslab != nullptr, "fused decoder tail: the weight-gradient slab pool is exhausted");
        x.db = w.d3; x.red = w.red_d[2];
        WgradSlabJob j{};
        const PackDesc& gd = P.gk.d[P.convT[3].gk[0]];
        j.dst = P.buf.gpk + gd.dst_off; j.slab = x.wslab; j.N = 32; j.K = 16; j.Kpad = gd.Kpad; j.chunks = chunks;
        j.chunk_stride = 32 * 16; j.src_ld = 16; j.stream = s;
        P.slab.jobs.push_back(j);
    }
    return launch_dec_last_fused(x, s);
}

int dec_fwd(MMPlan& P, int groups, int training, ConvTLastFwdArgs* last, hipStream_t s, int last_groups = -1, int fused_bwd_groups = -1,
            bool fuse = false) {
    MMPlan::W& w = P.w;
    const int B = P.B, rows = groups * B;
    {
        GatherPlan pl = dense_plan(rows, P.ldz, P.ldz, 1024);
        GemmParams g = gemm_of(P, pl, &P.up.pk_fwd, 1, rows);
        g.c.A = w.z_bf; g.out_bf = w.u; g.ldo = 1024; g.out_act_bf = w.au; g.e_act = ACT_SWISH;
        MMVAE_TRY(launch_gemm_gather(g, s));
    }
    bf16* q[4] = {w.u, w.q1, w.q2, w.q3};
    bf16* aq[4] = {w.au, w.aq1, w.aq2, w.aq3};
    for (int l = 0; l < 3; ++l) {
        const ConvL& L = P.convT[l];
        {
            GemmParams g = gemm_of(P, L.fwd, L.pk_fwd, groups, B, L.pk_fwd_f);
            g.c.A = aq[l];
            g.out_bf = q[l + 1]; g.ldo = L.g.Cout;
            g.colstats = training ? w.st_d[l] : nullptr;
            GatherTransform tr{};
            if (fuse && l >= 1) {
                const ConvL& Lp = P.convT[l - 1];
                const int prpg = B * Lp.g.OH * Lp.g.OW;
                tr.kind = 1;
                tr.fin = bn_fin_args(P, P.bn[Lp.bn], prpg, groups, w.st_d[l - 1], 1, w.aff_d[l - 1], w.mr_d[l - 1], training);
                g.c.A = q[l]; g.tr = &tr;
                if (mmvae_knob("mm_stage_out", 1)) tr.out = aq[l];
            }
            MMVAE_TRY(launch_gemm_gather(g, s));
        }
        const int rpg = B * L.g.OH * L.g.OW;
        if (l == 2 && fused_bwd_groups >= 0) continue;
        if (fuse && l <= 1) continue;
        MMVAE_TRY(bn_act(P, P.bn[L.bn], q[l + 1], aq[l + 1], groups * rpg, rpg, groups, w.st_d[l], 1, w.aff_d[l], w.mr_d[l], training, s));
    }
    if (fused_bwd_groups >= 0) return fused_tail(P, groups, training, last, last_groups, fused_bwd_groups, s);
    ConvTLastFwdArgs x = *last;
    x.act = w.aq3; x.w = P.buf.params + P.convT[3].w_off; x.G = last_groups > 0 ? last_groups : groups; x.B = B; x.IH = 25; x.IW = 25; x.Cin = 32; x.Cout = 1;
    return launch_convt_last_fwd(x, s);
}

int dec_bwd(MMPlan& P, const float* dlogit, int groups, float* dz, hipStream_t s, bool last_fused = false, bool fuse = false,
            int fwd_groups = 0, int training = 1) {
    MMPlan::W& w = P.w;
    const int B = P.B, rows = groups * B;
    bf16* q[4] = {w.u, w.q1, w.q2, w.q3};
    bf16* aq[4] = {w.au, w.aq1, w.aq2, w.aq3};
    bf16* dq[4] = {w.du, w.d1, w.d2, w.d3};
    bf16* dqr[4] = {nullptr, w.d1r, w.d2r, w.d3r};
    if (last_fused) {
        if (P.wgrad_forked) {
            PlanBase* pb = &P;
            side_later(P, [pb, s](hipStream_t wst) {
                for (WgradSlabJob& j : pb->slab.jobs) if (j.stream == s && j.src_ld == 16) j.stream = wst;
                return launch_wgrad_reduce(&pb->slab, wst, true);
            });
        }
    } else {
        const ConvL& L = P.convT[3];
        MMVAE_TRY(launch_im2col_small(dlogit, rows, 1, IMG, IMG, 4, 4, 2, 1, 25, 25, w.patches4, 16, s));
        {
            GatherPlan pd = dense_plan(B * 625, 16, 16, 32);
            GemmParams d = gemm_of(P, pd, L.pk_dgrad, groups, B * 625);
            d.c.A = w.patches4; d.out_bf = w.d3; d.ldo = 32;
            d.d_r = w.q3; d.d_ld = 32; d.d_act = ACT_SWISH; d.d_affine = w.aff_d[2]; d.d_meanrstd = w.mr_d[2]; d.d_red = w.red_d[2];
            arm_fork(P);
            MMVAE_TRY(launch_gemm_gather(d, s));
            MMVAE_TRY(commit_fork(P, s));
        }
        GatherPlan pl = plan_fwdform(1, 1, 25, 25, 16, 1, 1, 1, 0, 32, groups, B);
        WgradParams g = wgrad_of(P, pl, L.gk, groups, B);
        g.c.A = w.patches4; g.c.AH = 25; g.c.AW = 25; g.c.sy = g.c.sx = 1;
        g.P = w.aq3; g.ldp = 32;
        MMVAE_TRY(wgrad_async(P, g, s));
    }
    for (int l = 2; l >= 0; --l) {
        const ConvL& L = P.convT[l];
        const BnL& b = P.bn[L.bn];
        const int pix = L.g.OH * L.g.OW;
        const bool fl = fuse;
        BnBwdApplyArgs x{};
        x.db = dq[l + 1]; x.r = q[l + 1]; x.dr = fl ? dqr[l + 1] : dq[l + 1]; x.rows = rows * pix; x.C = L.g.Cout; x.ld = L.g.Cout;
        x.rows_per_group = B * pix; x.G = groups;
        x.red = w.red_d[l]; x.meanrstd = w.mr_d[l]; x.gamma = P.buf.params + b.w_off;
        x.dgamma = P.buf.grads + b.w_off; x.dbeta = P.buf.grads + b.b_off;
        if (!fl) MMVAE_TRY(launch_bn_bwd_apply(x, s));
        WgradParams gw = convT_wgrad(P, L, groups, B, aq[l], x.dr);
        if (fl) {
            MMPlan* pp = &P;
            const ConvL& Lp = P.convT[l >= 1 ? l - 1 : 0];
            const int prpg = B * Lp.g.OH * Lp.g.OW;
            {
                const bool byp = mmvae_knob("mm_stage_out", 1) != 0;
                const bool actp = l >= 1 && !byp;
                const BnL bp = P.bn[Lp.bn];
                const bf16* qin = q[l]; bf16* aqo = aq[l]; const float2* st = w.st_d[l >= 1 ? l - 1 : 0];
                side_later(P, [pp, x, gw, byp, actp, bp, qin, aqo, st, groups, prpg, training](hipStream_t ws_) {
                    if (!byp) MMVAE_TRY(launch_bn_bwd_apply(x, ws_));
                    if (actp) MMVAE_TRY(bn_act_side(*pp, bp, qin, aqo, groups * prpg, prpg, groups, st, training, ws_));
                    return wgrad_on(*pp, gw, ws_);
                });
            }
        } else if (fuse || l == 0) {
            MMPlan* pp = &P;
            side_later(P, [pp, gw](hipStream_t ws_) { return wgrad_on(*pp, gw, ws_); });
        }
        {
            GemmParams d = gemm_of(P, L.dgrad, L.pk_dgrad, groups, B, L.pk_dgrad_f);
            d.c.A = dq[l + 1]; d.out_bf = dq[l]; d.ldo = L.g.Cin;
            d.d_r = q[l]; d.d_ld = L.g.Cin; d.d_act = ACT_SWISH;
            if (l > 0) { d.d_affine = w.aff_d[l - 1]; d.d_meanrstd = w.mr_d[l - 1]; d.d_red = w.red_d[l - 1]; }
            GatherTransform tr{};
            if (fl) {
                tr.kind = 2; tr.r = q[l + 1]; tr.red = w.red_d[l]; tr.mr = w.mr_d[l]; tr.gamma = P.buf.params + b.w_off;
                tr.inv_cnt = 1.f / (float)(B * pix); tr.groups = groups;
                if (mmvae_knob("mm_stage_out", 1)) { tr.out = dqr[l + 1]; tr.dgamma = P.buf.grads + b.w_off; tr.dbeta = P.buf.grads + b.b_off; }
                d.tr = &tr;
            }
            const bool flush = P.wgrad_forked && ((l == 2 && !mmvae_knob("mm_forks", 0)) || l == 0);
            if (flush) arm_fork(P);
            MMVAE_TRY(launch_gemm_gather(d, s));
            if (flush) { MMVAE_TRY(commit_fork(P, s)); if (l == 2) MMVAE_TRY(side_flush(P, s)); }
        }
        if (!fl && !(fuse || l == 0)) MMVAE_TRY(wgrad_async(P, gw, s));
    }
    {
        GatherPlan pl = dense_plan(rows, P.ldz, P.ldz, 1024);
        WgradParams g = wgrad_of(P, pl, &P.up.gk, 1, rows);
        g.c.A = w.z_bf; g.P = w.du; g.ldp = 1024;
        MMPlan* pp = &P;
        side_later(P, [pp, g](hipStream_t ws_) { return wgrad_on(*pp, g, ws_); });
        MMVAE_TRY(side_flush(P, s));
        GatherPlan pd = dense_plan(rows, 1024, 1024, P.D);
        GemmParams d = gemm_of(P, pd, &P.up.pk_dgrad, 1, rows);
        d.c.A = w.du; d.out_f = dz; d.ldo = P.D;
        MMVAE_TRY(launch_gemm_gather(d, s));
    }
    return MMVAE_OK;
}

GruPacked gru_of(const MMPlan& P, const MMPlan::GruIdx& g) {
    GruPacked r{};
    r.wih = P.buf.packed + P.pk.d[g.wih].dst_off; r.kih = P.pk.d[g.wih].Kpad;
    r.whh = P.buf.packed + P.pk.d[g.whh].dst_off;
    r.wihT = P.buf.packed + P.pk.d[g.wihT].dst_off; r.nih = P.pk.d[g.wihT].Npad;
    r.whhT = P.buf.packed + P.pk.d[g.whhT].dst_off;
    r.bih = P.buf.params + g.bih; r.bhh = P.buf.params + g.bhh;
    return r;
}
TextEncArgs te_args(MMPlan& P, const long long* text, float* out, bool save) {
    MMPlan::W& w = P.w;
    TextEncArgs a{};
    a.B = P.B; a.D = P.D; a.tokens = text; a.embed = P.buf.params + off(P, "text_encoder.embed.weight");
    a.fwd = gru_of(P, P.te_f); a.rev = gru_of(P, P.te_r);
    a.h2p = P.buf.packed + P.pk.d[P.te_h2p].dst_off; a.nh2p = P.pk.d[P.te_h2p].Npad;
    a.h2pT = P.buf.packed + P.pk.d[P.te_h2pT].dst_off;
    a.h2p_bias = P.buf.params + off(P, "text_encoder.h2p.bias");
    a.out = out;
    if (save) { a.gates_f = w.te_gates_f; a.gates_r = w.te_gates_r; a.x_bf = w.te_x; a.hprev_bf = w.te_hprev; a.hsum_bf = w.te_hsum; }
    return a;
}
int txt_enc_bwd(MMPlan& P, const long long* text, const float* d_out, hipStream_t s) {
    MMPlan::W& w = P.w;
    const int B = P.B, D2 = 2 * P.D;
    TextEncBwdArgs a{};
    a.f = te_args(P, text, nullptr, true);
    a.d_out = d_out; a.d_out_bf = w.te_dout_bf;
    a.dgi_f = w.te_dgi_f; a.dgh_f = w.te_dgh_f; a.dgi_r = w.te_dgi_r;
    float* G = P.buf.grads;
    a.g_embed = G + off(P, "text_encoder.embed.weight");
    a.g_bih_f = G + P.te_f.bih; a.g_bhh_f = G + P.te_f.bhh; a.g_bih_r = G + P.te_r.bih; a.g_bhh_r = G + P.te_r.bhh;
    a.g_h2p_bias = G + off(P, "text_encoder.h2p.bias");
    MMVAE_TRY(launch_text_encoder_bwd(a, s));
    WgradParams list[4];
    int nl = 0;
    auto wg = [&](int gidx, const bf16* Pm, int N, int ldp, const bf16* Gm, int C, int rows) {
        GatherPlan pl = dense_plan(rows, C, C, N);
        WgradParams g = wgrad_of(P, pl, &gidx, 1, rows);
        g.c.A = Gm; g.P = Pm; g.ldp = ldp;
        list[nl++] = g;
    };
    wg(P.te_f.g_wih, w.te_dgi_f, 300, 304, w.te_x, TXT_HP, 4 * B);
    wg(P.te_f.g_whh, w.te_dgh_f, 300, 304, w.te_hprev, TXT_HP, 4 * B);
    wg(P.te_r.g_wih, w.te_dgi_r, 300, 304, w.te_x + (size_t)3 * B * TXT_HP, TXT_HP, B);
    wg(P.g_te_h2p, w.te_dout_bf, D2, round_up(D2, 8), w.te_hsum, TXT_HP, B);
    MMVAE_TRY(launch_wgrad_group(list, nl, s, &P.slab));
    return launch_wgrad_reduce(&P.slab, s, true);
}
TextDecArgs td_args(MMPlan& P, const float* z, int groups, bool save) {
    MMPlan::W& w = P.w;
    TextDecArgs a{};
    a.R = groups * P.B; a.D = P.D; a.rows_per_pass = P.B; a.z = z;
    a.embed = P.buf.params + off(P, "text_decoder.embed.weight");
    a.z2h = P.buf.packed + P.pk.d[P.td_z2h].dst_off; a.kz = P.kz;
    a.z2hT = P.buf.packed + P.pk.d[P.td_z2hT].dst_off;
    a.z2h_bias = P.buf.params + off(P, "text_decoder.z2h.bias");
    a.l0 = gru_of(P, P.td0); a.l1 = gru_of(P, P.td1);
    a.h2o = P.buf.packed + P.pk.d[P.td_h2o].dst_off; a.kx = P.kx;
    a.h2oT = P.buf.packed + P.pk.d[P.td_h2oT].dst_off;
    a.h2o_bias = P.buf.params + off(P, "text_decoder.h2o.bias");
    a.words = w.words; a.tokens_out = w.tokens;
    if (save) {
        a.gates = w.td_gates; a.x0_bf = w.td_x0; a.h0p_bf = w.td_h0p; a.mid_bf = w.td_mid; a.h1p_bf = w.td_h1p;
        a.hz_bf = w.td_hz; a.z_bf = w.td_zbf;
    }
    return a;
}
int txt_dec_bwd(MMPlan& P, const TextDecArgs& f, const float* dwords, float* dz, hipStream_t s) {
    MMPlan::W& w = P.w;
    const int R = f.R, XI = 100 + P.D;
    TextDecBwdArgs a{};
    a.f = f; a.dwords = dwords; a.R_active = R; a.dz = dz;
    a.dgi0 = w.dgi0; a.dgh0 = w.dgh0; a.dgi1 = w.dgi1; a.dgh1 = w.dgh1; a.dlogit_bf = w.dlogit_bf; a.dhinit_bf = w.dhinit;
    float* G = P.buf.grads;
    a.g_embed = G + off(P, "text_decoder.embed.weight");
    a.g_b[0] = G + P.td0.bih; a.g_b[1] = G + P.td0.bhh; a.g_b[2] = G + P.td1.bih; a.g_b[3] = G + P.td1.bhh;
    a.g_h2o_bias = G + off(P, "text_decoder.h2o.bias"); a.g_z2h_bias = G + off(P, "text_decoder.z2h.bias");
    P.ev_dz = nullptr;
    const bool own_ev = P.in_step && s == P.st_text && mmvae_knob("mm_dz_event", 1) != 0;
    if (own_ev) {
        P.ev_dz = next_ev(P);
        if (!P.capturing && !mmvae_knob("no_stop_events", 0)) mmvae_arm_stop_event(P.ev_dz);
    }
    MMVAE_TRY(launch_text_decoder_bwd(a, s));
    if (own_ev && (mmvae_take_stop_event() != nullptr || P.capturing || mmvae_knob("no_stop_events", 0)) && hipEventRecord(P.ev_dz, s) != hipSuccess) {
        mmvae_set_error("text decoder event failed: %s", hipGetErrorString(hipGetLastError()));
        return MMVAE_EHIP;
    }
    WgradParams list[6];
    int nl = 0;
    auto wg = [&](int gidx, const bf16* Pm, int N, int ldp, const bf16* Gm, int C, int rows) {
        GatherPlan pl = dense_plan(rows, C, C, N);
        WgradParams g = wgrad_of(P, pl, &gidx, 1, rows);
        g.c.A = Gm; g.P = Pm; g.ldp = ldp;
        list[nl++] = g;
    };
    (void)XI;
    wg(P.td0.g_wih, w.dgi0, 300, 304, w.td_x0, P.kx, 4 * R);
    wg(P.td0.g_whh, w.dgh0, 300, 304, w.td_h0p, TXT_HP, 4 * R);
    wg(P.td1.g_wih, w.dgi1, 300, 304, w.td_mid, TXT_HP, 4 * R);
    wg(P.td1.g_whh, w.dgh1, 300, 304, w.td_h1p, TXT_HP, 4 * R);
    wg(P.g_td_z2h, w.dhinit, 100, 112, w.td_zbf, P.kz, R);
    wg(P.g_td_h2o, w.dlogit_bf, 12, 16, w.td_hz, P.kx, 4 * R);
    MMVAE_TRY(launch_wgrad_group(list, nl, s, &P.slab));
    MMVAE_TRY(launch_wgrad_reduce(&P.slab, s, true));
    P.ev_txtgrads = nullptr;
    if (own_ev) {
        P.ev_txtgrads = next_ev(P);
        if (hipEventRecord(P.ev_txtgrads, s) != hipSuccess) {
            mmvae_set_error("text decoder event failed: %s", hipGetErrorString(hipGetLastError()));
            return MMVAE_EHIP;
        }
    }
    return MMVAE_OK;
}

}

MMPlan* mm_create(int D, int B) {
    if (D < 1 || D > 127 || B < 1) { mmvae_set_error("mm_create: need 1 <= n_latents <= 127 and batch >= 1"); return nullptr; }
    MMPlan* P = new MMPlan();
    P->D = D; P->B = B;
    P->single_wgrad_stream = true;
    build_plan(*P);
    plan_size_workspaces(*P, carve);
    return P;
}
void mm_destroy(MMPlan* P) { delete P; }
int mm_early_ranges(const MMPlan* P, long long* ranges, int cap) {
    int n = 0;
    for (const ParamInfo& pi : P->params) {
        if (pi.name.rfind("image_decoder.", 0) != 0 && pi.name.rfind("text_decoder.", 0) != 0) continue;
        if (n > 0 && ranges[2 * (n - 1)] + ranges[2 * (n - 1) + 1] == pi.offset) { ranges[2 * (n - 1) + 1] += pi.numel; continue; }
        if (n == cap) return 0;
        ranges[2 * n] = pi.offset; ranges[2 * n + 1] = pi.numel; ++n;
    }
    for (int r = 0; r < n; ++r)
        if (ranges[2 * r] % 4 != 0 || ranges[2 * r + 1] % 4 != 0) return 0;
    return n;
}
PlanBase* mm_base(MMPlan* P) { return P; }

static int use_ws(MMPlan* P, void* ws, size_t bytes, bool module = true) { return plan_use_ws(P, ws, bytes, module, carve); }

static int mm_step_body(MMPlan* Pp, const mmvae_mm_step_io& io, int training, int do_backward, hipStream_t s);
int mm_step_fwd_bwd(MMPlan* Pp, const mmvae_mm_step_io& io, int training, int do_backward, hipStream_t s) {
    if (const mmvae_early_adam* e = io.early_adam) {
        MMVAE_REQUIRE(e->m && e->v && e->state && e->gmap && e->ran, "mmvae_mm_step: early_adam with a null field");
        *e->ran = 0;
    }
    return plan_step(Pp, io, training, do_backward, s, mm_step_body);
}
static int mm_step_body(MMPlan* Pp, const mmvae_mm_step_io& io, int training, int do_backward, hipStream_t s) {
    MMVAE_TRY(use_ws(Pp, io.ws, io.ws_bytes, false));
    MMPlan& P = *Pp;
    MMPlan::W& w = P.w;
    const int B = P.B, D = P.D, B3 = 3 * B;
    MMVAE_REQUIRE(io.image && io.text && io.sums, "step: image/text/sums must be given");
    const float* eps = io.eps;
    const uint8_t *m1 = io.enc_mask1, *m2 = io.enc_mask2, *gk = io.gru_keep;
    const bool serial0 = mmvae_serial();
    const bool staged = mmvae_knob("mm_stage_begin", 1) != 0 && !serial0;
    StepBeginArgs sb{}, sb2{};
    sb.zero_ptr[0] = w.zero_begin; sb.zero_bytes[0] = w.zero_bytes;
    StepBeginArgs& sz = staged ? sb2 : sb;
    if (do_backward) {
        sz.zero_ptr[1] = P.buf.gpk; sz.zero_bytes[1] = (size_t)P.gk.mat_elems * sizeof(float);
        sz.zero_ptr[2] = P.buf.grads; sz.zero_bytes[2] = (size_t)(P.nparams / 4) * 16;
        const int skipz = mmvae_knob("dbg_begin_skip_zero", 0);
        if (skipz & 1) sz.zero_ptr[1] = nullptr;
        if (skipz & 2) sz.zero_ptr[2] = nullptr;
    }
    sb.p = DROP_P; sb.seed = io.seed; sb.step = io.step_counter;
    if (training && !eps) { sb.eps = w.eps; sb.n_eps = (long long)B3 * D; eps = w.eps; }
    if (training && io.enc_dropout && !m1) { sb.mask[0] = w.m1; sb.n_mask[0] = (long long)2 * B * 400; m1 = w.m1; }
    if (training && io.enc_dropout && !m2) { sb.mask[1] = w.m2; sb.n_mask[1] = (long long)2 * B * 200; m2 = w.m2; }
    if (training && io.gru_dropout && !gk) { sb.mask[2] = w.gkeep; sb.n_mask[2] = (long long)4 * B3 * 100; gk = w.gkeep; }
    const int skipb = mmvae_knob("dbg_begin_skip", 0);
    if (skipb & 2) { sb.eps = nullptr; sb.mask[0] = sb.mask[1] = sb.mask[2] = nullptr; }
    if (skipb & 4) sb.zero_ptr[0] = nullptr;
    const bool pack_now = io.pack_first && !(skipb & 1);
    if (pack_now) {
        MMVAE_TRY(step_begin_with_pack(sb, P.buf.desc_dev, P.pk.d.data(), (int)P.pk.d.size(), P.buf.params, P.buf.packed, P.buf.packed_vec));
        if (staged) sb.pack_parts = 1u << 0;
    }
    MMVAE_TRY(ensure_streams(P));
    P.in_step = true;
    {
        hipStreamCaptureStatus cs = hipStreamCaptureStatusNone;
        P.capturing = hipStreamIsCapturing(s, &cs) == hipSuccess && cs == hipStreamCaptureStatusActive;
    }
    arm_fork(P);
    MMVAE_TRY(launch_step_begin(sb, s));
    MMVAE_TRY(commit_fork(P, s));
    if (do_backward && P.nparams % 4 != 0)
        MMVAE_TRY(launch_fill_zero(P.buf.grads + (P.nparams / 4) * 4, (size_t)(P.nparams % 4) * sizeof(float), s));
    const int enc_drop = training && io.enc_dropout;
    const int sk[3] = {io.pass_skip[0] != 0, io.pass_skip[1] != 0, io.pass_skip[2] != 0};
    P.dec_skip_mask = (unsigned)(sk[0] | (sk[1] << 1) | (sk[2] << 2));
    const int enc_updates = 2 - sk[0] - sk[1];
    const bool serial = mmvae_serial();
    hipStream_t T = serial ? s : P.st_text;
    if (T != s) MMVAE_TRY(fork_to(P, T));
    if (staged && pack_now) {
        StepBeginArgs st1{};
        MMVAE_TRY(step_begin_with_pack(st1, P.buf.desc_dev, P.pk.d.data(), (int)P.pk.d.size(), P.buf.params, P.buf.packed, P.buf.packed_vec));
        st1.pack_parts = 1u << 1;
        MMVAE_TRY(launch_step_begin(st1, T));
    }
    {
        TextEncArgs a = te_args(P, io.text, w.txtout, do_backward);
        MMVAE_TRY(launch_text_encoder_fwd(a, T));
    }
    if (staged && (pack_now || sb2.zero_ptr[1] || sb2.zero_ptr[2])) {
        if (pack_now) {
            MMVAE_TRY(step_begin_with_pack(sb2, P.buf.desc_dev, P.pk.d.data(), (int)P.pk.d.size(), P.buf.params, P.buf.packed, P.buf.packed_vec));
            sb2.pack_parts = 1u << 2;
        }
        MMVAE_TRY(launch_step_begin(sb2, T));
    }
    P.step_image = io.image;
    const bool fuse = mmvae_knob("mm_fuse_bn", 1) != 0 && mmvae_knob("convres", 1) != 0 && B % 8 == 0;
    MMVAE_TRY(enc_fwd(P, io.image, 2, m1, m2, enc_drop, training, enc_updates, w.encout, s, fuse));
    MMVAE_TRY(edge(P, T, s));
    Latent3Args la{};
    la.B = B; la.D = D; la.img_out = w.encout; la.txt_out = w.txtout; la.eps = eps;
    la.mu = io.mu ? io.mu : w.mu; la.logvar = io.logvar ? io.logvar : w.logvar;
    la.z_f32 = w.z_f32; la.z_bf = w.z_bf; la.ldz = P.ldz; la.kl_sum = w.sums + 8; la.training = training;
    arm_fork(P);
    MMVAE_TRY(launch_latent3_fwd(la, s));
    MMVAE_TRY(commit_fork(P, s));
    if (T != s) MMVAE_TRY(fork_to(P, T));
    TextDecArgs td = td_args(P, w.z_f32, 3, do_backward);
    td.keep = (training && io.gru_dropout) ? gk : nullptr; td.keep_scale = 1.f / (1.f - DROP_P);
    td.force_tokens = io.force_tokens;
    if (io.recon_text) td.words = io.recon_text;
    if (io.tokens) td.tokens_out = io.tokens;
    td.target = io.text; td.nll_sum = w.sums + 4; td.dwords = do_backward ? w.dwords : nullptr;
    for (int k = 0; k < 3; ++k) td.nll_coef[k] = sk[k] ? 0.f : io.lambda_yx[k] / (float)(B * TXT_T);
    if (const int half = mmvae_knob("dbg_text_rows_div", 0)) td.R = max(16, td.R / half);
    MMVAE_TRY(launch_text_decoder_fwd(td, T));
    if (do_backward) MMVAE_TRY(txt_dec_bwd(P, td, w.dwords, w.dz_txt, T));
    ConvTLastFwdArgs last{};
    last.target = io.image; last.recon = io.recon_image; last.dlogit = do_backward ? w.dlogit : nullptr; last.loss_sum = w.sums;
    for (int k = 0; k < 3; ++k) last.coef[k] = sk[k] ? 0.f : io.lambda_xy[k] / (float)(B * NPIX);
    int last_groups = 3;
    if (!io.recon_image)
        while (last_groups > 1 && last.coef[last_groups - 1] == 0.f) --last_groups;
    int img_groups = 3;
    while (img_groups > 0 && (io.lambda_xy[img_groups - 1] == 0.f || sk[img_groups - 1])) --img_groups;
    const bool fuse_tail = P.slab.pool != nullptr;
    MMVAE_TRY(dec_fwd(P, 3, training, &last, s, last_groups, fuse_tail ? (do_backward ? std::min(img_groups, last_groups) : 0) : -1, fuse));
    if (!do_backward) {
        MMVAE_TRY(edge(P, T, s));
        P.in_step = false;
        hipLaunchKernelGGL(sum_slots_kernel, dim3(1), dim3(64), 0, s, w.sums, io.sums);
        return mmvae_check_launch("sum_slots");
    }

    P.wgrad_forked = mmvae_knob("mm_wgrad_inline", 0) == 0;
    int rc = MMVAE_OK;
    P.deferred.clear();
    P.defer_wgrad = false;
    if (img_groups > 0) rc = dec_bwd(P, w.dlogit, img_groups, w.dz_img, s, fuse_tail, fuse, 3, training);
    if (io.early_adam && rc == MMVAE_OK && img_groups > 0 && fuse && fuse_tail && P.wgrad_forked && !serial && T != s && !io.dp_split &&
        io.defer_unpack && P.ev_txtgrads && P.side_pending.empty() && P.st_wgrad2 == P.st_wgrad && mmvae_knob("mm_early_adam", 1)) {
        hipStream_t Wst = P.st_wgrad;
        AdamArgs ad{};
        const mmvae_early_adam& ea = *io.early_adam;
        ad.p = P.buf.params; ad.g = P.buf.grads; ad.m = ea.m; ad.v = ea.v; ad.n = P.nparams; ad.step = ea.state;
        ad.lr = ea.lr; ad.b1 = ea.beta1; ad.b2 = ea.beta2; ad.eps = ea.eps; ad.grad_scale = ea.grad_scale;
        ad.gmap = ea.gmap; ad.gpk = P.buf.gpk; ad.gpk_vec = P.buf.gpk_vec; ad.g_out = P.buf.grads;
        long long rg[8];
        ad.nr = mm_early_ranges(&P, rg, 4);
        for (int r = 0; r < ad.nr; ++r) { ad.roff[r] = rg[2 * r]; ad.rlen[r] = rg[2 * r + 1]; }
        ad.no_advance = 1;
        if (ad.nr > 0) {
            if (hipStreamWaitEvent(Wst, P.ev_txtgrads, 0) != hipSuccess) { mmvae_set_error("early optimizer part: %s", hipGetErrorString(hipGetLastError())); rc = MMVAE_EHIP; }
            if (rc == MMVAE_OK) rc = launch_adam(ad, Wst);
            if (rc == MMVAE_OK) *ea.ran = 1;
        }
    }
    if (rc == MMVAE_OK) {
        const int k = mmvae_knob("dbg_skip_edges", 0);
        if (P.ev_dz && T != s) {
            if (k != 1 && k != 3 && hipStreamWaitEvent(s, P.ev_dz, 0) != hipSuccess) {
                mmvae_set_error("stream join failed: %s", hipGetErrorString(hipGetLastError()));
                rc = MMVAE_EHIP;
            }
        } else {
            rc = edge(P, T, s);
        }
    }
    const bool dp_split = io.dp_split && !io.defer_unpack;
    if (dp_split && rc == MMVAE_OK) {
        rc = edge(P, s, T);
        if (rc == MMVAE_OK && P.st_wgrad != T) rc = edge(P, P.st_wgrad, T);
        if (rc == MMVAE_OK && P.st_wgrad2 != P.st_wgrad && P.st_wgrad2 != T) rc = edge(P, P.st_wgrad2, T);
        if (rc == MMVAE_OK) rc = launch_wgrad_reduce(&P.slab, T);
        if (rc == MMVAE_OK)
            rc = plan_unpack(P, T, false, 1);
        if (rc == MMVAE_OK) {
            if (!P.ev_early) hipEventCreateWithFlags(&P.ev_early, hipEventDisableTiming);
            if (hipEventRecord(P.ev_early, T) != hipSuccess) { mmvae_set_error("early-gradient event failed"); rc = MMVAE_EHIP; }
        }
    }
    Latent3BwdArgs lb{};
    lb.f = la; lb.dz_a = w.dz_img; lb.dz_b = w.dz_txt;
    for (int k = 0; k < 3; ++k) lb.kl_coef[k] = sk[k] ? 0.f : io.kl_lambda / (float)B;
    lb.d_img_out_bf = w.d_encout; lb.d_img_bias = P.buf.grads + P.fc[2].b_off; lb.d_txt_out = w.d_txtout;
    lb.loss_slots = w.sums; lb.loss_out = io.sums;
    if (rc == MMVAE_OK) {
        arm_fork(P);
        rc = launch_latent3_bwd(lb, s);
        if (rc == MMVAE_OK) rc = commit_fork(P, s);
    }
    if (rc == MMVAE_OK) rc = flush_wgrads(P, s);
    if (rc == MMVAE_OK && T != s) rc = fork_to(P, T);
    if (rc == MMVAE_OK) rc = txt_enc_bwd(P, io.text, w.d_txtout, T);
    if (rc == MMVAE_OK) rc = enc_bwd(P, w.d_encout, 2, m1, m2, enc_drop, s, fuse);
    P.wgrad_forked = false;
    P.in_step = false;
    MMVAE_TRY(rc);
    MMVAE_TRY(join_sides(P, T, s));
    MMVAE_TRY(launch_wgrad_reduce(&P.slab, s));
    if (dp_split) return plan_unpack(P, s, false, 0);
    if (!io.defer_unpack) MMVAE_TRY(plan_unpack(P, s, true));
    return MMVAE_OK;
}
int mm_wait_early_grads(MMPlan* P, hipStream_t s) {
    MMVAE_REQUIRE(P && P->ev_early, "mm_wait_early_grads: no dp_split step has run on this plan");
    if (hipStreamWaitEvent(s, P->ev_early, 0) != hipSuccess) {
        mmvae_set_error("mm_wait_early_grads: %s", hipGetErrorString(hipGetLastError()));
        return MMVAE_EHIP;
    }
    return MMVAE_OK;
}

int mm_image_encoder_fwd(MMPlan* P, void* ws, size_t wsb, const float* image, const uint8_t* m1, const uint8_t* m2,
                         int training, float* out, hipStream_t s) {
    MMVAE_TRY(use_ws(P, ws, wsb));
    MMPlan::W& w = P->w;
    MMVAE_TRY(launch_fill_zero(w.zero_begin, w.zero_bytes, s));
    return enc_fwd(*P, image, 1, m1, m2, training && m1 != nullptr, training, 1, out, s);
}
int mm_image_encoder_bwd(MMPlan* P, void* ws, size_t wsb, const float* d_out, const uint8_t* m1, const uint8_t* m2, hipStream_t s) {
    MMVAE_TRY(use_ws(P, ws, wsb));
    MMPlan::W& w = P->w;
    const int rows = P->B, D2 = 2 * P->D;
    MMVAE_TRY(plan_zero_gpk(*P, s));
    hipLaunchKernelGGL(cast_bf_kernel, dim3(ceil_div(rows * D2, 256)), dim3(256), 0, s, d_out, (long long)rows * D2, w.d_encout);
    hipLaunchKernelGGL(colsum_kernel, dim3(ceil_div(D2, 64)), dim3(64), 0, s, d_out, rows, D2, P->buf.grads + P->fc[2].b_off);
    MMVAE_TRY(mmvae_check_launch("image encoder bwd prologue"));
    MMVAE_TRY(enc_bwd(*P, w.d_encout, 1, m1, m2, m1 != nullptr, s));
    return plan_unpack(*P, s, true);
}
int mm_image_decoder_fwd(MMPlan* P, void* ws, size_t wsb, const float* z, int training, float* recon, hipStream_t s) {
    MMVAE_TRY(use_ws(P, ws, wsb));
    MMPlan::W& w = P->w;
    const int rows = P->B;
    MMVAE_TRY(launch_fill_zero(w.zero_begin, w.zero_bytes, s));
    hipLaunchKernelGGL(cast_z_kernel, dim3(ceil_div(rows * P->ldz, 256)), dim3(256), 0, s, z, rows, P->D, w.z_bf, P->ldz);
    MMVAE_TRY(mmvae_check_launch("cast_z"));
    ConvTLastFwdArgs last{};
    last.recon = recon;
    return dec_fwd(*P, 1, training, &last, s);
}
int mm_image_decoder_bwd(MMPlan* P, void* ws, size_t wsb, const float* d_recon, const float* recon, float* dz, hipStream_t s) {
    MMVAE_TRY(use_ws(P, ws, wsb));
    MMPlan::W& w = P->w;
    const int rows = P->B;
    MMVAE_TRY(plan_zero_gpk(*P, s));
    hipLaunchKernelGGL(sigmoid_bwd_kernel, dim3(ceil_div(rows * NPIX, 256)), dim3(256), 0, s, d_recon, recon, (long long)rows * NPIX, w.dlogit);
    MMVAE_TRY(mmvae_check_launch("sigmoid_bwd"));
    MMVAE_TRY(dec_bwd(*P, w.dlogit, 1, dz, s));
    return plan_unpack(*P, s, true);
}
int mm_text_encoder_fwd(MMPlan* P, void* ws, size_t wsb, const long long* text, float* out, hipStream_t s) {
    MMVAE_TRY(use_ws(P, ws, wsb));
    TextEncArgs a = te_args(*P, text, out, true);
    return launch_text_encoder_fwd(a, s);
}
int mm_text_encoder_bwd(MMPlan* P, void* ws, size_t wsb, const long long* text, const float* d_out, hipStream_t s) {
    MMVAE_TRY(use_ws(P, ws, wsb));
    MMVAE_TRY(plan_zero_gpk(*P, s));
    MMVAE_TRY(txt_enc_bwd(*P, text, d_out, s));
    return plan_unpack(*P, s, true);
}
int mm_text_decoder_fwd(MMPlan* P, void* ws, size_t wsb, const float* z, int training, const uint8_t* keep,
                        const long long* force_tokens, float* words, long long* tokens, hipStream_t s) {
    MMVAE_TRY(use_ws(P, ws, wsb));
    TextDecArgs a = td_args(*P, z, 1, true);
    a.keep = training ? keep : nullptr; a.keep_scale = 1.f / (1.f - DROP_P);
    a.force_tokens = force_tokens; a.words = words; a.tokens_out = tokens;
    return launch_text_decoder_fwd(a, s);
}
int mm_text_decoder_bwd(MMPlan* P, void* ws, size_t wsb, const float* z, const uint8_t* keep, const long long* force_tokens,
                        const float* words, const long long* tokens, const float* d_words, float* dz, hipStream_t s) {
    MMVAE_TRY(use_ws(P, ws, wsb));
    MMVAE_TRY(plan_zero_gpk(*P, s));
    TextDecArgs a = td_args(*P, z, 1, true);
    a.keep = keep; a.keep_scale = 1.f / (1.f - DROP_P);
    a.force_tokens = force_tokens; a.words = const_cast<float*>(words); a.tokens_out = const_cast<long long*>(tokens);
    MMVAE_TRY(txt_dec_bwd(*P, a, d_words, dz, s));
    return plan_unpack(*P, s, true);
}

int mm_iw_score(MMPlan* P, void* ws, size_t wsb, const float* z, const float* image, int B, int K, float* loglik_x, float* words,
                hipStream_t s) {
    MMVAE_REQUIRE(P && z && image && loglik_x && words, "mmvae_mm_iw_score: null argument");
    MMVAE_REQUIRE(B >= 1 && K >= 1 && (long long)B * K <= P->B,
                  "mmvae_mm_iw_score: %d examples x %d particles exceed the plan's %d rows", B, K, P->B);
    MMVAE_TRY(use_ws(P, ws, wsb));
    MMPlan::W& w = P->w;
    const int rows = B * K;
    MMVAE_TRY(launch_fill_zero(w.zero_begin, w.zero_bytes, s));
    hipLaunchKernelGGL(cast_z_kernel, dim3(ceil_div(rows * P->ldz, 256)), dim3(256), 0, s, z, rows, P->D, w.z_bf, P->ldz);
    MMVAE_TRY(mmvae_check_launch("cast_z"));
    ConvTLastFwdArgs last{};
    last.target = image; last.loglik = loglik_x; last.rows_per_target = K; last.rows = rows;
    MMVAE_TRY(dec_fwd(*P, 1, 0, &last, s, -1, 0));
    TextDecArgs a = td_args(*P, z, 1, false);
    a.R = rows; a.words = words;
    return launch_text_decoder_fwd(a, s);
}

static bool layer_gemm(MMPlan& P, const std::string& name, GemmParams& g) {
    MMPlan::W& w = P.w;
    const int B = P.B;
    bf16* r[4] = {w.r1, w.r2, w.r3, w.r4};
    bf16* a[4] = {w.a1, w.a2, w.a3, w.a4};
    bf16* dre[4] = {w.d1e, w.d2e, w.d3e, w.dr4};
    bf16* q[4] = {w.u, w.q1, w.q2, w.q3};
    bf16* aq[4] = {w.au, w.aq1, w.aq2, w.aq3};
    bf16* dq[4] = {w.du, w.d1, w.d2, w.d3};
    if (name == "enc_conv1") {
        GatherPlan pl = dense_plan(B * 625, 16, 16, 32);
        g = gemm_of(P, pl, P.conv[0].pk_fwd, 1, B * 625);
        g.c.A = w.patches1; g.out_bf = w.r1; g.ldo = 32; g.out_act_bf = w.a1; g.e_act = ACT_SWISH;
        return true;
    }
    for (int l = 1; l < 4; ++l) {
        const ConvL& L = P.conv[l];
        if (name == "enc_conv" + std::to_string(l + 1)) {
            g = gemm_of(P, L.fwd, L.pk_fwd, 1, B, L.pk_fwd_f);
            g.c.A = a[l - 1];
            g.out_bf = r[l]; g.ldo = L.g.Cout; g.colstats = w.st_e[l - 1];
            return true;
        }
        if (name == "enc_conv" + std::to_string(l + 1) + "_dgrad") {
            g = gemm_of(P, L.dgrad, L.pk_dgrad, 1, B, L.pk_dgrad_f);
            g.c.A = dre[l]; g.out_bf = dre[l - 1]; g.ldo = L.g.Cin;
            g.d_r = r[l - 1]; g.d_ld = L.g.Cin; g.d_act = ACT_SWISH;
            if (l > 1) { g.d_affine = w.aff_e[l - 2]; g.d_meanrstd = w.mr_e[l - 2]; g.d_red = w.red_e[l - 2]; }
            return true;
        }
    }
    {
        const int rows = 2 * B;
        const float ms = 1.f / (1.f - DROP_P);
        if (name == "enc_fc1") {
            GatherPlan pl = plan_fwdform(2, 2, 1, 1, 256, 2, 2, 1, 0, 400, 1, rows);
            g = gemm_of(P, pl, &P.fc[0].pk_fwd, 1, rows);
            g.c.A = w.a4; g.c.a_bcast_n = B; g.bias = P.buf.params + P.fc[0].b_off; g.out_bf = w.y1; g.ldo = 400;
            g.out_act_bf = w.ay1; g.e_act = ACT_SWISH; g.e_mask = w.m1; g.e_mask_scale = ms;
            return true;
        }
        if (name == "enc_fc2") {
            GatherPlan pl = dense_plan(rows, 400, 400, 200);
            g = gemm_of(P, pl, &P.fc[1].pk_fwd, 1, rows);
            g.c.A = w.ay1; g.bias = P.buf.params + P.fc[1].b_off; g.out_bf = w.y2; g.ldo = 200;
            g.out_act_bf = w.ay2; g.e_act = ACT_SWISH; g.e_mask = w.m2; g.e_mask_scale = ms;
            return true;
        }
        if (name == "enc_fc3") {
            GatherPlan pl = dense_plan(rows, 200, 200, 2 * P.D);
            g = gemm_of(P, pl, &P.fc[2].pk_fwd, 1, rows);
            g.c.A = w.ay2; g.bias = P.buf.params + P.fc[2].b_off; g.out_f = w.tmp_f32; g.ldo = 2 * P.D;
            return true;
        }
        if (name == "enc_fc3_dgrad") {
            GatherPlan pd = dense_plan(rows, 2 * P.D, 2 * P.D, 200);
            g = gemm_of(P, pd, &P.fc[2].pk_dgrad, 1, rows);
            g.c.A = w.d_encout; g.out_bf = w.dy2; g.ldo = 200;
            g.d_r = w.y2; g.d_ld = 200; g.d_act = ACT_SWISH; g.d_mask = w.m2; g.d_mask_scale = ms;
            g.d_colsum = w.tmp_f32;
            return true;
        }
        if (name == "enc_fc2_dgrad") {
            GatherPlan pd = dense_plan(rows, 200, 200, 400);
            g = gemm_of(P, pd, &P.fc[1].pk_dgrad, 1, rows);
            g.c.A = w.dy2; g.out_bf = w.dy1; g.ldo = 400;
            g.d_r = w.y1; g.d_ld = 400; g.d_act = ACT_SWISH; g.d_mask = w.m1; g.d_mask_scale = ms;
            g.d_colsum = w.tmp_f32;
            return true;
        }
        if (name == "dec_up") {
            GatherPlan pl = dense_plan(3 * B, P.ldz, P.ldz, 1024);
            g = gemm_of(P, pl, &P.up.pk_fwd, 1, 3 * B);
            g.c.A = w.z_bf; g.out_bf = w.u; g.ldo = 1024; g.out_act_bf = w.au; g.e_act = ACT_SWISH;
            return true;
        }
        if (name == "dec_up_dgrad") {
            GatherPlan pd = dense_plan(rows, 1024, 1024, P.D);
            g = gemm_of(P, pd, &P.up.pk_dgrad, 1, rows);
            g.c.A = w.du; g.out_f = w.tmp_f32; g.ldo = P.D;
            return true;
        }
    }
    if (name == "dec_last_dgrad_gemm") {
        const ConvL& L = P.convT[3];
        GatherPlan pl = dense_plan(B * 625, 16, 16, 32);
        g = gemm_of(P, pl, L.pk_dgrad, 2, B * 625);
        g.c.A = w.patches4; g.out_bf = w.d3; g.ldo = 32;
        g.d_r = w.q3; g.d_ld = 32; g.d_act = ACT_SWISH; g.d_affine = w.aff_d[2]; g.d_meanrstd = w.mr_d[2]; g.d_red = w.red_d[2];
        return true;
    }
    for (int l = 0; l < 3; ++l) {
        const ConvL& L = P.convT[l];
        if (name == "dec_convT" + std::to_string(l + 1)) {
            g = gemm_of(P, L.fwd, L.pk_fwd, 3, B, L.pk_fwd_f);
            g.c.A = aq[l];
            g.out_bf = q[l + 1]; g.ldo = L.g.Cout; g.colstats = w.st_d[l];
            return true;
        }
        if (name == "dec_convT" + std::to_string(l + 1) + "_dgrad") {
            g = gemm_of(P, L.dgrad, L.pk_dgrad, 2, B, L.pk_dgrad_f);
            g.c.A = dq[l + 1]; g.out_bf = dq[l]; g.ldo = L.g.Cin;
            g.d_r = q[l]; g.d_ld = L.g.Cin; g.d_act = ACT_SWISH;
            if (l > 0) { g.d_affine = w.aff_d[l - 1]; g.d_meanrstd = w.mr_d[l - 1]; g.d_red = w.red_d[l - 1]; }
            return true;
        }
    }
    return false;
}
static bool layer_wgrad(MMPlan& P, const std::string& name, WgradParams& g) {
    MMPlan::W& w = P.w;
    const int B = P.B;
    bf16* a[4] = {w.a1, w.a2, w.a3, w.a4};
    bf16* dre[4] = {w.d1e, w.d2e, w.d3e, w.dr4};
    bf16* aq[4] = {w.au, w.aq1, w.aq2, w.aq3};
    bf16* dq[4] = {w.du, w.d1, w.d2, w.d3};
    for (int l = 0; l < 3; ++l)
        if (name == "dec_convT" + std::to_string(l + 1) + "_wgrad") {
            const ConvL& L = P.convT[l];
            g = convT_wgrad(P, L, 2, B, aq[l], dq[l + 1]);
            return true;
        }
    for (int l = 1; l < 4; ++l)
        if (name == "enc_conv" + std::to_string(l + 1) + "_wgrad") {
            const ConvL& L = P.conv[l];
            g = wgrad_of(P, L.fwd, L.gk, 1, B);
            g.c.A = a[l - 1]; g.P = dre[l]; g.ldp = L.g.Cout;
            return true;
        }
    if (name == "dec_last_wgrad") {
        GatherPlan pl = plan_fwdform(1, 1, 25, 25, 16, 1, 1, 1, 0, 32, 2, B);
        g = wgrad_of(P, pl, P.convT[3].gk, 2, B);
        g.c.A = w.patches4; g.c.AH = 25; g.c.AW = 25; g.c.sy = g.c.sx = 1;
        g.P = w.aq3; g.ldp = 32;
        return true;
    }
    if (name == "enc_conv1_wgrad") {
        GatherPlan pl = dense_plan(B * 625, 16, 16, 32);
        g = wgrad_of(P, pl, P.conv[0].gk, 1, B * 625);
        g.c.A = w.patches1; g.P = w.d1e; g.ldp = 32;
        return true;
    }
    return false;
}
static double wgrad_flops(const WgradParams& g) {
    double f = 0;
    for (int i = 0; i < g.c.nclasses; ++i) f += 2.0 * g.c.groups * g.cls[i].rows_per_group * (double)g.c.N * g.cls[i].K;
    return f;
}
static double gemm_flops(const GemmParams& g) {
    double f = 0;
    for (int i = 0; i < g.c.nclasses; ++i) f += 2.0 * g.c.groups * g.cls[i].rows_per_group * (double)g.c.N * g.cls[i].K;
    return f;
}
int mm_bench_layer(MMPlan* P, void* ws, size_t wsb, const char* layer, int iters, hipStream_t s) {
    MMVAE_TRY(use_ws(P, ws, wsb, false));
    if (std::string(layer) == "dec_last_fused") {
        ConvTLastFwdArgs last{};
        last.target = (const float*)P->w.tmp_f32; last.loss_sum = P->w.sums;
        last.coef[0] = last.coef[1] = 1.f / (float)(P->B * NPIX);
        for (int i = 0; i < iters; ++i) {
            P->slab.reset(P->w.slab, P->w.slab_floats);
            MMVAE_TRY(fused_tail(*P, 3, 1, &last, 2, 2, s));
            P->slab.jobs.clear(); P->slab.ring_jobs.clear();
        }
        return MMVAE_OK;
    }
    WgradParams wg{};
    if (layer_wgrad(*P, layer, wg)) {
        for (int i = 0; i < iters; ++i) {
            P->slab.reset(P->w.slab, P->w.slab_floats);
            MMVAE_TRY(launch_wgrad(wg, s, &P->slab));
            MMVAE_TRY(launch_wgrad_reduce(&P->slab, s));
        }
        return MMVAE_OK;
    }
    GemmParams g{};
    MMVAE_REQUIRE(layer_gemm(*P, layer, g), "bench_layer: unknown layer '%s'", layer);
    for (int i = 0; i < iters; ++i) MMVAE_TRY(launch_gemm_gather(g, s));
    return MMVAE_OK;
}
double mm_layer_flops(const MMPlan* Pc, const char* layer) {
    MMPlan& P = *const_cast<MMPlan*>(Pc);
    GemmParams g{};
    WgradParams wg{};
    if (std::string(layer) == "dec_last_fused") return 3.0 * 2.0 * 2 * P.B * 625 * 16 * 32;
    if (P.bound && layer_wgrad(P, layer, wg)) return wgrad_flops(wg);
    if (!P.bound || !layer_gemm(P, layer, g)) return -1.0;
    return gemm_flops(g);
}
double mm_layer_algo_flops(const MMPlan* Pc, const char* layer) {
    const MMPlan& P = *Pc;
    const std::string name = layer;
    const int B = P.B;
    auto conv = [&](const ConvL& L, int images) {
        const ConvGeom& g = L.g;
        const double pix = g.transposed ? (double)g.IH * g.IW : (double)g.OH * g.OW;
        return 2.0 * pix * g.KH * g.KW * g.Cin * g.Cout * images;
    };
    for (int l = 0; l < 4; ++l) {
        const std::string e = "enc_conv" + std::to_string(l + 1), d = "dec_convT" + std::to_string(l + 1);
        if (name == e || name == e + "_dgrad" || name == e + "_wgrad") return conv(P.conv[l], B);
        if (name == d) return conv(P.convT[l], 3 * B);
        if (name == d + "_dgrad" || name == d + "_wgrad") return conv(P.convT[l], 2 * B);
    }
    if (name == "dec_last_wgrad" || name == "dec_last_dgrad_gemm") return conv(P.convT[3], 2 * B);
    return mm_layer_flops(Pc, layer);
}
double mm_layer_algo_bytes(const MMPlan* Pc, const char* layer) {
    const MMPlan& P = *Pc;
    const std::string name = layer;
    const int B = P.B;
    auto conv = [&](const ConvL& L, int images, bool wgrad) {
        const ConvGeom& g = L.g;
        const double act = (double)images * ((double)g.IH * g.IW * g.Cin + (double)g.OH * g.OW * g.Cout) * 2.0;
        return act + (double)g.Cin * g.Cout * g.KH * g.KW * (wgrad ? 4.0 : 2.0);
    };
    for (int l = 0; l < 4; ++l) {
        const std::string e = "enc_conv" + std::to_string(l + 1), d = "dec_convT" + std::to_string(l + 1);
        if (name == e || name == e + "_dgrad") return conv(P.conv[l], B, false);
        if (name == e + "_wgrad") return conv(P.conv[l], B, true);
        if (name == d) return conv(P.convT[l], 3 * B, false);
        if (name == d + "_dgrad") return conv(P.convT[l], 2 * B, false);
        if (name == d + "_wgrad") return conv(P.convT[l], 2 * B, true);
    }
    return 0.0;
}
long long mm_debug_offset(MMPlan* P, const char* name) {
    Workspace ws((void*)0x1000, (size_t)1 << 40);
    P->carve_passes = 3;
    carve(*P, ws);
    MMPlan::W& w = P->w;
    std::map<std::string, const void*> m = {
        {"patches1", w.patches1}, {"r1", w.r1}, {"r2", w.r2}, {"r3", w.r3}, {"r4", w.r4}, {"y1", w.y1}, {"y2", w.y2},
        {"encout", w.encout}, {"txtout", w.txtout}, {"z_bf", w.z_bf}, {"z_f32", w.z_f32}, {"u", w.u}, {"q1", w.q1}, {"q2", w.q2},
        {"q3", w.q3}, {"logits", w.logits}, {"dlogit", w.dlogit}, {"d3", w.d3}, {"d2", w.d2}, {"d1", w.d1}, {"du", w.du},
        {"dz_img", w.dz_img}, {"dz_txt", w.dz_txt}, {"d_encout", w.d_encout}, {"d_txtout", w.d_txtout}, {"dy2", w.dy2},
        {"dy1", w.dy1}, {"db4", w.db4}, {"dr4", w.dr4}, {"d3e", w.d3e}, {"d2e", w.d2e}, {"d1e", w.d1e},
        {"aff_d0", w.aff_d[0]}, {"aff_d1", w.aff_d[1]}, {"aff_d2", w.aff_d[2]}, {"st_d0", w.st_d[0]}, {"patches4", w.patches4},
        {"tmp_f32", w.tmp_f32}, {"aff_e0", w.aff_e[0]}, {"aff_e1", w.aff_e[1]}, {"aff_e2", w.aff_e[2]},
        {"eps", w.eps}, {"m1", w.m1}, {"m2", w.m2}, {"gkeep", w.gkeep},
        {"st_e0", w.st_e[0]}, {"st_e1", w.st_e[1]}, {"st_e2", w.st_e[2]}, {"st_d1", w.st_d[1]}, {"st_d2", w.st_d[2]},
        {"red_e0", w.red_e[0]}, {"red_e1", w.red_e[1]}, {"red_e2", w.red_e[2]},
        {"red_d0", w.red_d[0]}, {"red_d1", w.red_d[1]}, {"red_d2", w.red_d[2]},
        {"a1", w.a1}, {"a2", w.a2}, {"a3", w.a3}, {"aq1", w.aq1}, {"aq2", w.aq2}, {"aq3", w.aq3},
        {"a4", w.a4}, {"au", w.au}, {"ay1", w.ay1}, {"ay2", w.ay2}, {"slab", w.slab},
        {"mr_e0", w.mr_e[0]}, {"mr_e1", w.mr_e[1]}, {"mr_e2", w.mr_e[2]}, {"mr_d0", w.mr_d[0]}, {"mr_d1", w.mr_d[1]}, {"mr_d2", w.mr_d[2]},
    };
    auto it = m.find(name);
    if (it == m.end()) return -1;
    return (long long)((const char*)it->second - (const char*)0x1000);
}
```

Before: 1714 ELBO-steps/s.

## Make conv-residual kernels persistent with LDS-resident weights and atomic batch tickets

Adds a persistent mode to the convres kernel. Each workgroup loops over image batches, taking the next batch from an atomic ticket counter or a static stride, and prefetches the next batch's input during the current compute. In WRES mode all weight classes are loaded into LDS once per workgroup rather than streamed chunk by chunk for each batch, and setup work such as tables, BN constants and buffer descriptors is hoisted out of the batch loop. It is enabled by default for conv2, convT3 and conv2 dgrad. The aim is to cut repeated weight traffic and per-block launch and setup cost, at the price of more LDS per block, possible lower occupancy, and ticket atomics.

```diff
diff --git a/multimodal-vae_amd/csrc/convres.hip b/multimodal-vae_amd/csrc/convres.hip
--- a/multimodal-vae_amd/csrc/convres.hip
+++ b/multimodal-vae_amd/csrc/convres.hip
@@ -40,6 +40,7 @@
     float t_inv_cnt;
     int t_groups;
     bf16* stage_out;
+    unsigned* ticket;
     unsigned long long* ts;
 };
 
@@ -52,7 +53,7 @@
     return r;
 }
 
-template <class G, int NI, int CH, int WAVES, int NG, bool SCR_OWN, int NSPLIT = 1, int KSPL = 1>
+template <class G, int NI, int CH, int WAVES, int NG, bool SCR_OWN, int NSPLIT = 1, int KSPL = 1, bool WRES = false>
 struct CrLayout {
     static constexpr int NTHR = WAVES * 64;
     static constexpr int MG = WAVES / (NG * KSPL), NT = G::N / 32 / NSPLIT / NG;
@@ -60,23 +61,29 @@
     static constexpr int RED_BYTES = KSPL > 1 ? WAVES * max_mt() * NT * 4096 : 0;
     static constexpr bool BDIR = CH == 0;
     static constexpr int BP = (CH * 16 + 8) * 2;
-    static constexpr int W_BYTES = BDIR ? 0 : G::N * BP;
+    static constexpr int wpitch(int c) { return WRES ? G::K(c) * 2 + 16 : BP; }
+    static constexpr int w_off(int c) { int o = 0; for (int i = 0; i < c; ++i) o += G::N * wpitch(i); return WRES ? o : 0; }
+    static constexpr int W_BYTES = BDIR ? 0 : WRES ? w_off(G::NCLS) : G::N * BP;
     static_assert(!BDIR || SCR_OWN, "direct-B kernels have no weight buffer to lend to the epilogue");
+    static_assert(!WRES || (SCR_OWN && !BDIR), "resident weights are never lent to the epilogue");
     static constexpr int IMG_ALL = NI * G::IMG_BYTES;
     static constexpr int TAB_BYTES = tab_base<G, NI>(G::NCLS) * 4;
     static constexpr int SCR_PITCH = 80, SCR_BYTES = 32 * SCR_PITCH;
     static constexpr int TRT_BYTES = G::C * 16;
     static constexpr int OFF_W = IMG_ALL, OFF_TAB = OFF_W + W_BYTES, OFF_TRT = OFF_TAB + TAB_BYTES,
-                         OFF_SCR = OFF_TRT + TRT_BYTES, OFF_RED = OFF_SCR + (SCR_OWN ? WAVES * SCR_BYTES : 0), TOTAL = OFF_RED + RED_BYTES;
+                         OFF_SCR = OFF_TRT + TRT_BYTES, OFF_RED = OFF_SCR + (SCR_OWN ? WAVES * SCR_BYTES : 0), OFF_NXT = OFF_RED + RED_BYTES,
+                         TOTAL = OFF_NXT + 16;
     static_assert((NSPLIT == 1 && KSPL == 1) || BDIR, "column / k splits exist for the direct-B kernels only");
     static_assert(G::N % (32 * NSPLIT * NG) == 0 && WAVES % (NG * KSPL) == 0, "wave decomposition");
     static_assert(SCR_OWN || W_BYTES >= WAVES * SCR_BYTES, "the weight buffer doubles as the epilogue scratch");
     static_assert(TOTAL <= 160 * 1024, "LDS budget");
 };
 
-template <class G, int NI, int CH, int WAVES, int NG, bool SCR_OWN, int MODE, int TR, int NSPLIT = 1, int KSPL = 1>
+template <class G, int NI, int CH, int WAVES, int NG, bool SCR_OWN, int MODE, int TR, int NSPLIT = 1, int KSPL = 1, int PM = 0>
 __global__ __launch_bounds__(WAVES * 64) void convres_kernel(const ConvResArgs a) {
-    using L = CrLayout<G, NI, CH, WAVES, NG, SCR_OWN, NSPLIT, KSPL>;
+    constexpr bool PERSIST = PM != 0, WRES = PM == 2;
+    static_assert(!PERSIST || NSPLIT == 1, "the batches of a persistent launch are dealt over gridDim.x alone");
+    using L = CrLayout<G, NI, CH, WAVES, NG, SCR_OWN, NSPLIT, KSPL, WRES>;
     constexpr int NT = L::NT, MG = L::MG, NTHR = WAVES * 64;
     constexpr int BP = L::BP, SCR_PITCH = L::SCR_PITCH;
     extern __shared__ __attribute__((aligned(16))) char smem[];
@@ -84,21 +91,24 @@
     char* const w_s = smem + L::OFF_W;
     unsigned* const tab = reinterpret_cast<unsigned*>(smem + L::OFF_TAB);
     float4* const trt = reinterpret_cast<float4*>(smem + L::OFF_TRT);
+    int& next_bat_s = *reinterpret_cast<int*>(smem + L::OFF_NXT);
 
     const int tid = threadIdx.x, lane = tid & 63;
     const int wave = __builtin_amdgcn_readfirstlane(tid >> 6);
     const int r = lane & 31, h = lane >> 5;
     const int kg = wave % KSPL, ng = (wave / KSPL) % NG, mg = wave / (KSPL * NG);
     const int ntb = blockIdx.y * (G::N / 32 / NSPLIT) + ng * NT;
-    const int img0 = blockIdx.x * NI;
-    const int grp = img0 / a.group_n;
+    const int nbat = a.nimg / NI;
+    int bat = blockIdx.x;
+    int img0 = bat * NI;
+    int grp = img0 / a.group_n;
     auto stamp = [&](int idx) {
         if (a.ts && lane == 0) a.ts[((size_t)blockIdx.x * WAVES + wave) * 16 + idx] = __builtin_amdgcn_s_memrealtime();
     };
     stamp(0);
 
     constexpr bool BDIR = L::BDIR;
-    constexpr int WV = BDIR ? 1 : crgeo::cdiv(G::N * CH * 2, NTHR);
+    constexpr int WV = (BDIR || WRES) ? 1 : crgeo::cdiv(G::N * CH * 2, NTHR);
     i32x4c wreg[WV];
     auto w_fetch = [&](auto ci, auto chi) {
         constexpr int c = decltype(ci)::value, ch = decltype(chi)::value;
@@ -122,17 +132,18 @@
             if (v < NV) *reinterpret_cast<i32x4c*>(w_s + n * BP + kv * 16) = wreg[it];
         }
     };
-    if constexpr (!BDIR) w_fetch(std::integral_constant<int, 0>{}, std::integral_constant<int, 0>{});
+    if constexpr (!BDIR && !WRES) w_fetch(std::integral_constant<int, 0>{}, std::integral_constant<int, 0>{});
 
     constexpr int VPP = G::C / 8;
     constexpr int NVI = NI * G::AH * G::AW * VPP;
     constexpr int IT = crgeo::cdiv(NVI, NTHR), SB = 4, NB = crgeo::cdiv(IT, SB);
+    constexpr size_t IMG_ELEMS = (size_t)G::AH * G::AW * G::C;
     static_assert(NTHR % VPP == 0, "a thread keeps its channel vector across staging iterations");
-    const bf16* const src = a.A + (size_t)img0 * (G::AH * G::AW * G::C);
-    const bf16* const src_r = TR == 2 ? a.t_r + (size_t)img0 * (G::AH * G::AW * G::C) : nullptr;
-    bf16* const stage_dst = (TR != 0 && a.stage_out && blockIdx.y == 0) ? a.stage_out + (size_t)img0 * (G::AH * G::AW * G::C) : nullptr;
+    const bool stage_wr = TR != 0 && a.stage_out && blockIdx.y == 0;
     i32x4c ireg[SB], rreg[TR == 2 ? SB : 1];
-    auto i_fetch = [&](int b) {
+    auto i_fetch = [&](int b, int first_img) {
+        const bf16* const src = a.A + (size_t)first_img * IMG_ELEMS;
+        const bf16* const src_r = TR == 2 ? a.t_r + (size_t)first_img * IMG_ELEMS : nullptr;
 #pragma unroll
         for (int i = 0; i < SB; ++i) {
             const int v = tid + (b * SB + i) * NTHR;
@@ -144,6 +155,7 @@
     };
     float tc0[TR ? 8 : 1], tc1[TR ? 8 : 1], tc2[TR == 2 ? 8 : 1];
     auto i_store = [&](int b) {
+        bf16* const stage_dst = stage_wr ? a.stage_out + (size_t)img0 * IMG_ELEMS : nullptr;
 #pragma unroll
         for (int i = 0; i < SB; ++i) {
             const int v = tid + (b * SB + i) * NTHR;
@@ -172,7 +184,29 @@
             }
         }
     };
-    if (!(a.dbg & 4)) i_fetch(0);
+    if (!(a.dbg & 4)) i_fetch(0, img0);
+
+    auto make_trt = [&]() {
+        if constexpr (TR == 1) {
+            for (int ch = tid; ch < G::C; ch += NTHR) {
+                float2 aff, mr;
+                bn_channel_tables(a.fin, grp, ch, aff, mr);
+                trt[ch] = make_float4(aff.x, aff.y, 0.f, 0.f);
+            }
+        } else if constexpr (TR == 2) {
+            for (int ch = tid; ch < G::C; ch += NTHR) {
+                float sx = 0.f, sy = 0.f;
+                for (int q = 0; q < MMVAE_STAT_SLOTS; ++q) {
+                    const float2 t = a.t_red[((size_t)grp * MMVAE_STAT_SLOTS + q) * G::C + ch];
+                    sx += t.x; sy += t.y;
+                }
+                const float2 mr = a.t_mr[grp * G::C + ch];
+                const float g = a.t_gamma[ch] * mr.y, m1 = sx * a.t_inv_cnt, m2 = sy * a.t_inv_cnt;
+                const float cb = -g * m2 * mr.y;
+                trt[ch] = make_float4(g, cb, -cb * mr.x - g * m1, 0.f);
+            }
+        }
+    };
 
     {
         const i32x4c z = {0, 0, 0, 0};
@@ -191,12 +225,29 @@
                 tab[tab_base<G, NI>(c) + e] = v;
             }
         });
+        if constexpr (WRES) {
+            static_for<0, G::NCLS>([&](auto ci) {
+                constexpr int c = decltype(ci)::value;
+                constexpr int VPR = G::KSTEPS(c) * 2, NV = G::N * VPR, WB = 8;
+                const bf16* wsrc = a.Wp[c];
+                const int kpad = a.Kpad[c];
+                for (int v0 = tid; v0 < NV; v0 += WB * NTHR) {
+                    i32x4c t[WB];
+#pragma unroll
+                    for (int i = 0; i < WB; ++i) {
+                        const int v = v0 + i * NTHR, n = v / VPR, kv = v - n * VPR;
+                        if (v < NV) t[i] = *reinterpret_cast<const i32x4c*>(wsrc + (size_t)n * kpad + kv * 8);
+                    }
+#pragma unroll
+                    for (int i = 0; i < WB; ++i) {
+                        const int v = v0 + i * NTHR, n = v / VPR, kv = v - n * VPR;
+                        if (v < NV) *reinterpret_cast<i32x4c*>(w_s + L::w_off(c) + n * L::wpitch(c) + kv * 16) = t[i];
+                    }
+                }
+            });
+        }
+        make_trt();
         if constexpr (TR == 1) {
-            for (int ch = tid; ch < G::C; ch += NTHR) {
-                float2 aff, mr;
-                bn_channel_tables(a.fin, grp, ch, aff, mr);
-                trt[ch] = make_float4(aff.x, aff.y, 0.f, 0.f);
-            }
             if (blockIdx.x == 0 && blockIdx.y == 0) {
                 for (int i = tid; i < a.fin.G * G::C; i += NTHR) {
                     float2 aff, mr;
@@ -206,17 +257,6 @@
                 bn_running_update(a.fin, tid, NTHR);
             }
         } else if constexpr (TR == 2) {
-            for (int ch = tid; ch < G::C; ch += NTHR) {
-                float sx = 0.f, sy = 0.f;
-                for (int q = 0; q < MMVAE_STAT_SLOTS; ++q) {
-                    const float2 t = a.t_red[((size_t)grp * MMVAE_STAT_SLOTS + q) * G::C + ch];
-                    sx += t.x; sy += t.y;
-                }
-                const float2 mr = a.t_mr[grp * G::C + ch];
-                const float g = a.t_gamma[ch] * mr.y, m1 = sx * a.t_inv_cnt, m2 = sy * a.t_inv_cnt;
-                const float cb = -g * m2 * mr.y;
-                trt[ch] = make_float4(g, cb, -cb * mr.x - g * m1, 0.f);
-            }
             if (blockIdx.x == 0 && blockIdx.y == 0 && (a.t_dgamma || a.t_dbeta)) {
                 for (int ch = tid; ch < G::C; ch += NTHR) {
                     float tg = 0.f, tb = 0.f;
@@ -231,7 +271,52 @@
             }
         }
     }
+
+    const __amdgpu_buffer_rsrc_t orsrc = __builtin_amdgcn_make_buffer_rsrc(
+        a.out, 0, (int)((size_t)a.nimg * G::OH * G::OW * a.ldo * 2), 0x00020000);
+    const __amdgpu_buffer_rsrc_t rrsrc = __builtin_amdgcn_make_buffer_rsrc(
+        const_cast<bf16*>(a.d_r ? a.d_r : a.out), 0, (int)((size_t)a.nimg * G::OH * G::OW * a.ldo * 2), 0x00020000);
+    float dsc[NT], dsh[NT], dmean[NT], drstd[NT], s1[NT], s2[NT];
+    auto group_consts = [&]() {
+#pragma unroll
+        for (int nt = 0; nt < NT; ++nt) {
+            const int co = (ntb + nt) * 32 + r;
+            dsc[nt] = 1.f; dsh[nt] = 0.f; dmean[nt] = 0.f; drstd[nt] = 0.f; s1[nt] = 0.f; s2[nt] = 0.f;
+            if (MODE == 1 && a.d_affine) { const float2 t = a.d_affine[grp * G::N + co]; dsc[nt] = t.x; dsh[nt] = t.y; }
+            if (MODE == 1 && a.d_meanrstd) { const float2 t = a.d_meanrstd[grp * G::N + co]; dmean[nt] = t.x; drstd[nt] = t.y; }
+        }
+    };
+    group_consts();
+    auto flush_sums = [&]() {
+        float2* red = MODE == 1 ? a.d_red : a.colstats;
+        if (red && kg == 0) {
+            const int slot = (int)(blockIdx.x + wave) % MMVAE_STAT_SLOTS;
+#pragma unroll
+            for (int nt = 0; nt < NT; ++nt) {
+                const float t1 = s1[nt] + __shfl_xor(s1[nt], 32, 64), t2 = s2[nt] + __shfl_xor(s2[nt], 32, 64);
+                if (h == 0) {
+                    float2* d = red + ((size_t)grp * MMVAE_STAT_SLOTS + slot) * G::N + (ntb + nt) * 32 + r;
+                    atomicAdd(&d->x, t1);
+                    atomicAdd(&d->y, t2);
+                }
+            }
+        }
+    };
+    char* const scr = (SCR_OWN ? smem + L::OFF_SCR : w_s) + wave * L::SCR_BYTES;
+    __amdgpu_buffer_rsrc_t wrsrc[BDIR ? G::NCLS : 1];
+    if constexpr (BDIR) {
+#pragma unroll
+        for (int i = 0; i < G::NCLS; ++i)
+            wrsrc[i] = __builtin_amdgcn_make_buffer_rsrc(const_cast<bf16*>(a.Wp[i]), 0, a.Npad * a.Kpad[i] * 2, 0x00020000);
+    }
     stamp(1);
+
+    for (;;) {
+    int next_bat = nbat;
+    if constexpr (PERSIST) {
+        if (a.ticket) { if (tid == 0) next_bat = (int)gridDim.x + (int)atomicAdd(a.ticket, 1u); }
+        else next_bat = crgeo::persist_next(bat, (int)gridDim.x);
+    }
     __syncthreads();
     stamp(2);
     if constexpr (TR != 0) {
@@ -245,43 +330,30 @@
     }
     if (!(a.dbg & 4)) {
         i_store(0);
-        for (int b = 1; b < NB; ++b) { i_fetch(b); i_store(b); }
-    }
-    if constexpr (!BDIR) w_store(std::integral_constant<int, 0>{}, std::integral_constant<int, 0>{});
+        for (int b = 1; b < NB; ++b) { i_fetch(b, img0); i_store(b); }
+    }
+    if constexpr (!BDIR && !WRES) w_store(std::integral_constant<int, 0>{}, std::integral_constant<int, 0>{});
+    if constexpr (PERSIST) { if (a.ticket && tid == 0) next_bat_s = next_bat; }
     stamp(3);
     __syncthreads();
     stamp(4);
-
-    const __amdgpu_buffer_rsrc_t orsrc = __builtin_amdgcn_make_buffer_rsrc(
-        a.out, 0, (int)((size_t)a.nimg * G::OH * G::OW * a.ldo * 2), 0x00020000);
-    const __amdgpu_buffer_rsrc_t rrsrc = __builtin_amdgcn_make_buffer_rsrc(
-        const_cast<bf16*>(a.d_r ? a.d_r : a.out), 0, (int)((size_t)a.nimg * G::OH * G::OW * a.ldo * 2), 0x00020000);
+    if constexpr (PERSIST) {
+        if (a.ticket) next_bat = next_bat_s;
+        if (next_bat < nbat && !(a.dbg & 4)) i_fetch(0, next_bat * NI);
+    }
     const unsigned wg_out = (unsigned)img0 * (unsigned)(G::OH * G::OW) * (unsigned)a.ldo * 2u;
-    float dsc[NT], dsh[NT], dmean[NT], drstd[NT], s1[NT], s2[NT];
-#pragma unroll
-    for (int nt = 0; nt < NT; ++nt) {
-        const int co = (ntb + nt) * 32 + r;
-        dsc[nt] = 1.f; dsh[nt] = 0.f; dmean[nt] = 0.f; drstd[nt] = 0.f; s1[nt] = 0.f; s2[nt] = 0.f;
-        if (MODE == 1 && a.d_affine) { const float2 t = a.d_affine[grp * G::N + co]; dsc[nt] = t.x; dsh[nt] = t.y; }
-        if (MODE == 1 && a.d_meanrstd) { const float2 t = a.d_meanrstd[grp * G::N + co]; dmean[nt] = t.x; drstd[nt] = t.y; }
-    }
-    char* const scr = (SCR_OWN ? smem + L::OFF_SCR : w_s) + wave * L::SCR_BYTES;
-    __amdgpu_buffer_rsrc_t wrsrc[BDIR ? G::NCLS : 1];
-    if constexpr (BDIR) {
-#pragma unroll
-        for (int i = 0; i < G::NCLS; ++i)
-            wrsrc[i] = __builtin_amdgcn_make_buffer_rsrc(const_cast<bf16*>(a.Wp[i]), 0, a.Npad * a.Kpad[i] * 2, 0x00020000);
-    }
 
     static_for<0, G::NCLS>([&](auto ci) {
         constexpr int c = decltype(ci)::value;
         constexpr int ROWS = NI * G::OYX(c), T = crgeo::cdiv(ROWS, 32), MT = crgeo::cdiv(T, MG);
-        constexpr int KS = G::KSTEPS(c), CHE = BDIR ? KS : CH, NCH = crgeo::cdiv(KS, CHE);
+        constexpr int KS = G::KSTEPS(c), CHE = (BDIR || WRES) ? KS : CH, NCH = crgeo::cdiv(KS, CHE);
         constexpr int KSL = KS / KSPL;
+        constexpr int WP = L::wpitch(c);
+        const int mgc = WRES ? crgeo::persist_first_tile(mg, tab_base<G, NI>(c) / 32, MG) : mg;
         int abase[MT];
 #pragma unroll
         for (int m = 0; m < MT; ++m) {
-            const int t = mg + m * MG;
+            const int t = mgc + m * MG;
             int R = (t < T ? t : 0) * 32 + r;
             R = R < ROWS ? R : ROWS - 1;
             const int img = R / G::OYX(c), q = R - img * G::OYX(c);
@@ -300,8 +372,7 @@
             for (int nt = 0; nt < NT; ++nt)
 #pragma unroll
                 for (int j = 0; j < 16; ++j) acc[m][nt][j] = 0.f;
-        const int wrow = ((ng * NT) * 32 + r) * BP + h * 16;
-
+        const int wrow = L::w_off(c) + ((ng * NT) * 32 + r) * WP + h * 16;
         if constexpr (BDIR) {
             constexpr int PD = KSL < 8 ? KSL : 8;
             static_assert(KSPL == 1 || KSL % 2 == 0, "a wave's k range starts on a 32-column block of the packed weights");
@@ -381,7 +452,7 @@
             constexpr int ch = decltype(chi)::value;
             constexpr int CHK = crgeo::cmin(CHE, KS - ch * CHE);
             constexpr bool last_chunk = ch + 1 == NCH;
-            constexpr bool has_next = !BDIR && (!last_chunk || c + 1 < G::NCLS);
+            constexpr bool has_next = !BDIR && !WRES && (!last_chunk || c + 1 < G::NCLS);
             constexpr int cn = last_chunk ? c + 1 : c, chn = last_chunk ? 0 : ch + 1;
             if constexpr (has_next) w_fetch(std::integral_constant<int, cn>{}, std::integral_constant<int, chn>{});
             if (!BDIR && !(a.dbg & 2)) {
@@ -391,7 +462,7 @@
                     constexpr int aoff = G::step_off(c, ch * CHE + kk);
 #pragma unroll
                     for (int nt = 0; nt < NT; ++nt)
-                        fb[nt] = *reinterpret_cast<const bf16x8*>(w_s + wrow + nt * 32 * BP + kk * 32);
+                        fb[nt] = *reinterpret_cast<const bf16x8*>(w_s + wrow + nt * 32 * WP + kk * 32);
 #pragma unroll
                     for (int m = 0; m < MT; ++m) fa[m] = *reinterpret_cast<const bf16x8*>(img_s + abase[m] + aoff);
                 };
@@ -421,7 +492,7 @@
                 if constexpr (!SCR_OWN) __syncthreads();
 #pragma unroll
                 for (int m = 0; m < MT; ++m) {
-                    const int t = mg + m * MG;
+                    const int t = mgc + m * MG;
                     if (t < T && kg == 0) {
                         const unsigned* trow = tab + tab_base<G, NI>(c) + t * 32;
                         const unsigned off0 = trow[lane & 15], off1 = trow[16 + (lane & 15)];
@@ -449,17 +520,23 @@
     });
 
     stamp(13);
-    float2* red = MODE == 1 ? a.d_red : a.colstats;
-    if (red && kg == 0) {
-        const int slot = (int)(blockIdx.x + wave) % MMVAE_STAT_SLOTS;
-#pragma unroll
-        for (int nt = 0; nt < NT; ++nt) {
-            const float t1 = s1[nt] + __shfl_xor(s1[nt], 32, 64), t2 = s2[nt] + __shfl_xor(s2[nt], 32, 64);
-            if (h == 0) {
-                float2* d = red + ((size_t)grp * MMVAE_STAT_SLOTS + slot) * G::N + (ntb + nt) * 32 + r;
-                atomicAdd(&d->x, t1);
-                atomicAdd(&d->y, t2);
-            }
+    if (!PERSIST || next_bat >= nbat) break;
+    bat = next_bat;
+    img0 = bat * NI;
+    if constexpr (!BDIR && !WRES) w_fetch(std::integral_constant<int, 0>{}, std::integral_constant<int, 0>{});
+    const int g2 = img0 / a.group_n;
+    if (g2 != grp) {
+        flush_sums();
+        grp = g2;
+        make_trt();
+        group_consts();
+    }
+    }
+    flush_sums();
+    if constexpr (PERSIST) {
+        if (a.ticket && tid == 0 && atomicAdd(a.ticket + 1, 1u) == gridDim.x * gridDim.y - 1) {
+            __hip_atomic_store(a.ticket, 0u, __ATOMIC_RELAXED, __HIP_MEMORY_SCOPE_AGENT);
+            __hip_atomic_store(a.ticket + 1, 0u, __ATOMIC_RELAXED, __HIP_MEMORY_SCOPE_AGENT);
         }
     }
     stamp(14);
@@ -488,19 +565,27 @@
     return true;
 }
 
-template <class G, int NI, int CH, int WAVES, int NG, bool SCR_OWN, int MODE, int TR, int NSPLIT, int KSPL>
+template <class L>
+int persist_wgs(int nbat) {
+    const int forced = mmvae_knob("convres_persist_wgs", 0);
+    const int wgs = forced > 0 ? forced : mmvae_cu_count() * crgeo::cmax(1, crgeo::cmin(2, 160 * 1024 / L::TOTAL));
+    return wgs < nbat ? wgs : nbat;
+}
+
+template <class G, int NI, int CH, int WAVES, int NG, bool SCR_OWN, int MODE, int TR, int NSPLIT, int KSPL, int PM>
 int launch_cr_mode(const ConvResArgs& a, hipStream_t stream) {
-    using L = CrLayout<G, NI, CH, WAVES, NG, SCR_OWN, NSPLIT, KSPL>;
+    using L = CrLayout<G, NI, CH, WAVES, NG, SCR_OWN, NSPLIT, KSPL, PM == 2>;
     static std::atomic<unsigned> attr_set{0};
     if (mmvae_first_use_on_device(attr_set))
-        hipFuncSetAttribute(reinterpret_cast<const void*>(&convres_kernel<G, NI, CH, WAVES, NG, SCR_OWN, MODE, TR, NSPLIT, KSPL>),
+        hipFuncSetAttribute(reinterpret_cast<const void*>(&convres_kernel<G, NI, CH, WAVES, NG, SCR_OWN, MODE, TR, NSPLIT, KSPL, PM>),
                             hipFuncAttributeMaxDynamicSharedMemorySize, 160 * 1024);
-    MMVAE_LAUNCH((convres_kernel<G, NI, CH, WAVES, NG, SCR_OWN, MODE, TR, NSPLIT, KSPL>), dim3(a.nimg / NI, NSPLIT), dim3(WAVES * 64), L::TOTAL, stream, a);
+    const int nbat = a.nimg / NI;
+    MMVAE_LAUNCH((convres_kernel<G, NI, CH, WAVES, NG, SCR_OWN, MODE, TR, NSPLIT, KSPL, PM>), dim3(PM ? persist_wgs<L>(nbat) : nbat, NSPLIT), dim3(WAVES * 64), L::TOTAL, stream, a);
     MMVAE_TRY(mmvae_check_launch("convres"));
     return 1;
 }
 
-template <class G, int NI, int CH, int WAVES, int NG, bool SCR_OWN, int NSPLIT = 1, int KSPL = 1>
+template <class G, int NI, int CH, int WAVES, int NG, bool SCR_OWN, int NSPLIT = 1, int KSPL = 1, int PM = 0>
 int launch_cr(const GemmParams& p, hipStream_t stream) {
     const GatherCommon& c = p.c;
     const int nimg = c.groups * c.group_n;
@@ -517,6 +602,7 @@
     a.ts = reinterpret_cast<unsigned long long*>(((unsigned long long)(unsigned)mmvae_knob("convres_ts_hi", 0) << 32) |
                                                  (unsigned)mmvae_knob("convres_ts_lo", 0));
     a.d_r = p.d_r; a.d_affine = p.d_affine; a.d_meanrstd = p.d_meanrstd; a.d_red = p.d_red;
+    a.ticket = PM && mmvae_knob("convres_ticket", 1) ? p.cr_ticket : nullptr;
     const int kind = p.tr ? p.tr->kind : 0;
     MMVAE_REQUIRE(!(p.tr && p.tr->out == c.A) || NSPLIT == 1, "convres: an in-place staging by-product needs one workgroup per image tile");
     if (mmvae_probe_on()) {
@@ -530,17 +616,17 @@
         MMVAE_REQUIRE(a.fin.C == G::C && a.fin.G == c.groups && a.fin.affine && a.fin.meanrstd && a.fin.gamma && a.fin.beta,
                       "convres: BatchNorm tables of the staged operand do not match the layer");
         MMVAE_REQUIRE(!p.d_r, "convres: forward-type staging transform on a data-gradient launch");
-        return launch_cr_mode<G, NI, CH, WAVES, NG, SCR_OWN, 0, 1, NSPLIT, KSPL>(a, stream);
+        return launch_cr_mode<G, NI, CH, WAVES, NG, SCR_OWN, 0, 1, NSPLIT, KSPL, PM>(a, stream);
     }
     if (kind == 2) {
         const GatherTransform& t = *p.tr;
         MMVAE_REQUIRE(p.d_r && t.r && t.red && t.mr && t.gamma && t.groups == c.groups, "convres: BatchNorm-backward staging needs r / sums / tables");
         a.t_r = t.r; a.t_red = t.red; a.t_mr = t.mr; a.t_gamma = t.gamma; a.t_dgamma = t.dgamma; a.t_dbeta = t.dbeta;
         a.t_inv_cnt = t.inv_cnt; a.t_groups = t.groups; a.stage_out = t.out;
-        return launch_cr_mode<G, NI, CH, WAVES, NG, SCR_OWN, 1, 2, NSPLIT, KSPL>(a, stream);
-    }
-    return p.d_r ? launch_cr_mode<G, NI, CH, WAVES, NG, SCR_OWN, 1, 0, NSPLIT, KSPL>(a, stream)
-                 : launch_cr_mode<G, NI, CH, WAVES, NG, SCR_OWN, 0, 0, NSPLIT, KSPL>(a, stream);
+        return launch_cr_mode<G, NI, CH, WAVES, NG, SCR_OWN, 1, 2, NSPLIT, KSPL, PM>(a, stream);
+    }
+    return p.d_r ? launch_cr_mode<G, NI, CH, WAVES, NG, SCR_OWN, 1, 0, NSPLIT, KSPL, PM>(a, stream)
+                 : launch_cr_mode<G, NI, CH, WAVES, NG, SCR_OWN, 0, 0, NSPLIT, KSPL, PM>(a, stream);
 }
 
 bool features_ok(const GemmParams& p) {
@@ -554,11 +640,17 @@
     return true;
 }
 
-template <class G, int NI, int CH, int WAVES, int NG, bool SCR_OWN, int NSPLIT = 1, int KSPL = 1>
+template <class G, int NI, int CH, int WAVES, int NG, bool SCR_OWN, int NSPLIT = 1, int KSPL = 1, int PM = 0>
 int try_cr(const GemmParams& p, hipStream_t stream) {
     if (!geo_matches<G>(p)) return 0;
     if (p.c.group_n % NI != 0) return 0;
-    return launch_cr<G, NI, CH, WAVES, NG, SCR_OWN, NSPLIT, KSPL>(p, stream);
+    return launch_cr<G, NI, CH, WAVES, NG, SCR_OWN, NSPLIT, KSPL, PM>(p, stream);
+}
+template <class G, int NI_RULE, int NI, int CH, int WAVES, int NG, int PM>
+int try_cr_persist(const GemmParams& p, hipStream_t stream) {
+    if (!geo_matches<G>(p)) return 0;
+    if (p.c.group_n % NI_RULE != 0 || p.c.group_n % NI != 0) return 0;
+    return launch_cr<G, NI, CH, WAVES, NG, true, 1, 1, PM>(p, stream);
 }
 
 using crgeo::Geo;
@@ -575,6 +667,8 @@
 typedef Geo<1, 128, 64, 8, 8, 16, 16, 4, 4, 2, 1> G_ca_convT2;
 typedef Geo<1, 64, 32, 16, 16, 32, 32, 4, 4, 2, 1> G_ca_convT3;
 
+constexpr int CR_PERSIST_DEFAULT = 2 | 4 | 8;
+
 }
 
 int try_launch_convres(const GemmParams& p, hipStream_t stream) {
@@ -586,6 +680,11 @@
     int rc;
     const int nimg = p.c.groups * p.c.group_n;
     const int alt = mmvae_knob("convres_alt", 0);
+    const int pk = mmvae_knob("convres_persist", 1);
+    const int pm = pk == 1 ? CR_PERSIST_DEFAULT : pk;
+    if ((pm & 2) && (rc = try_cr_persist<G_mm_conv2, 1, 1, 16, 10, 2, 2>(p, stream)) != 0) return rc;
+    if ((pm & 4) && alt != 1 && (rc = try_cr_persist<G_mm_convT3, 2, 1, 16, 8, 1, 2>(p, stream)) != 0) return rc;
+    if ((pm & 8) && (rc = try_cr_persist<G_mm_conv2d, 1, 1, 16, 8, 1, 2>(p, stream)) != 0) return rc;
     if ((rc = try_cr<G_mm_conv2, 1, 16, 8, 2, true>(p, stream)) != 0) return rc;
     if (alt != 3) {
         if ((rc = try_cr<G_mm_conv3, 2, 0, 8, 4, true>(p, stream)) != 0) return rc;
@@ -603,6 +702,7 @@
         if ((rc = try_cr<G_mm_convT1, 8, 0, 6, 1, true, 4, 2>(p, stream)) != 0) return rc;
         if ((rc = try_cr<G_mm_conv4, 8, 0, 8, 2, true, 4, 4>(p, stream)) != 0) return rc;
     }
+    if ((pm & 16) && (rc = try_cr<G_mm_convT3d, 2, 10, 8, 2, false, 1, 1, 1>(p, stream)) != 0) return rc;
     if ((rc = try_cr<G_mm_convT3d, 2, 10, 8, 2, false>(p, stream)) != 0) return rc;
     if (mmvae_knob("convres_celeba", 1)) {
         if ((rc = try_cr<G_ca_conv2, 1, 16, 8, 2, true>(p, stream)) != 0) return rc;
diff --git a/multimodal-vae_amd/csrc/convres_geo.h b/multimodal-vae_amd/csrc/convres_geo.h
--- a/multimodal-vae_amd/csrc/convres_geo.h
+++ b/multimodal-vae_amd/csrc/convres_geo.h
@@ -6,6 +6,9 @@
 constexpr int fdiv(int a, int b) { return a >= 0 ? a / b : -((-a + b - 1) / b); }
 constexpr int cmax(int a, int b) { return a > b ? a : b; }
 constexpr int cmin(int a, int b) { return a < b ? a : b; }
+
+constexpr int persist_next(int bat, int nwg) { return bat + nwg; }
+constexpr int persist_first_tile(int mg, int tiles_before, int MG) { return (mg + MG - tiles_before % MG) % MG; }
 
 template <int FORM_, int C_, int N_, int AH_, int AW_, int OH_, int OW_, int KH_, int KW_, int S_, int PAD_, int PIXPAD_ = 16>
 struct Geo {
diff --git a/multimodal-vae_amd/csrc/gemm.h b/multimodal-vae_amd/csrc/gemm.h
--- a/multimodal-vae_amd/csrc/gemm.h
+++ b/multimodal-vae_amd/csrc/gemm.h
@@ -74,6 +74,7 @@
     int npad;
     const GatherTransform* tr;
     int d_cmod;
+    unsigned* cr_ticket;
 };
 
 struct WgradParams {
diff --git a/multimodal-vae_amd/csrc/multimnist.hip b/multimodal-vae_amd/csrc/multimnist.hip
--- a/multimodal-vae_amd/csrc/multimnist.hip
+++ b/multimodal-vae_amd/csrc/multimnist.hip
@@ -23,6 +23,7 @@
     int mt_w2, mt_w3, mt_w3t, mt_w2t;
     struct W {
         char* zero_begin; size_t zero_bytes;
+        unsigned* cr_ticket;
         float2 *st_e[3], *red_e[3], *st_d[3], *red_d[3];
         float* sums; float* dz_img; float* dz_txt;
         float2 *aff_e[3], *mr_e[3], *aff_d[3], *mr_d[3];
@@ -203,6 +204,7 @@
     for (int i = 0; i < 3; ++i) { w.st_d[i] = ws.take<float2>(3 * SS * dc[i]); w.red_d[i] = ws.take<float2>(3 * SS * dc[i]); }
     w.sums = ws.take<float>(16 * MMVAE_LOSS_SLOTS);
     P.sk_cnt = ws.take<unsigned>(1024);
+    w.cr_ticket = ws.take<unsigned>(32);
     w.dz_img = ws.take<float>(B3 * D);
     w.dz_txt = ws.take<float>(B3 * D);
     char* z1 = ws.take<char>(0);
@@ -274,7 +276,7 @@
     for (int l = 1; l < 4; ++l) {
         const ConvL& L = P.conv[l];
         GemmParams g = gemm_of(P, L.fwd, L.pk_fwd, 1, B, L.pk_fwd_f);
-        g.c.A = a[l - 1];
+        g.c.A = a[l - 1]; g.cr_ticket = w.cr_ticket + 2 * (l - 1);
         g.out_bf = r[l]; g.ldo = L.g.Cout;
         g.colstats = training ? w.st_e[l - 1] : nullptr;
         GatherTransform tr{};
@@ -448,6 +450,7 @@
         }
         {
             GemmParams d = gemm_of(P, L.dgrad, L.pk_dgrad, 1, B, L.pk_dgrad_f);
+            d.cr_ticket = w.cr_ticket + 2 * (3 + l - 1);
             d.c.A = dr[l]; d.out_bf = dr[l - 1]; d.ldo = L.g.Cin;
             d.d_r = r[l - 1]; d.d_ld = L.g.Cin; d.d_act = ACT_SWISH;
             if (l > 1) { d.d_affine = w.aff_e[l - 2]; d.d_meanrstd = w.mr_e[l - 2]; d.d_red = w.red_e[l - 2]; }
@@ -530,6 +533,7 @@
         const ConvL& L = P.convT[l];
         {
             GemmParams g = gemm_of(P, L.fwd, L.pk_fwd, groups, B, L.pk_fwd_f);
+            g.cr_ticket = w.cr_ticket + 2 * (6 + l);
             g.c.A = aq[l];
             g.out_bf = q[l + 1]; g.ldo = L.g.Cout;
             g.colstats = training ? w.st_d[l] : nullptr;
@@ -622,6 +626,7 @@
         }
         {
             GemmParams d = gemm_of(P, L.dgrad, L.pk_dgrad, groups, B, L.pk_dgrad_f);
+            d.cr_ticket = w.cr_ticket + 2 * (9 + l);
             d.c.A = dq[l + 1]; d.out_bf = dq[l]; d.ldo = L.g.Cin;
             d.d_r = q[l]; d.d_ld = L.g.Cin; d.d_act = ACT_SWISH;
             if (l > 0) { d.d_affine = w.aff_d[l - 1]; d.d_meanrstd = w.mr_d[l - 1]; d.d_red = w.red_d[l - 1]; }
@@ -1099,12 +1104,14 @@
         const ConvL& L = P.conv[l];
         if (name == "enc_conv" + std::to_string(l + 1)) {
             g = gemm_of(P, L.fwd, L.pk_fwd, 1, B, L.pk_fwd_f);
+            g.cr_ticket = w.cr_ticket + 2 * (l - 1);
             g.c.A = a[l - 1];
             g.out_bf = r[l]; g.ldo = L.g.Cout; g.colstats = w.st_e[l - 1];
             return true;
         }
         if (name == "enc_conv" + std::to_string(l + 1) + "_dgrad") {
             g = gemm_of(P, L.dgrad, L.pk_dgrad, 1, B, L.pk_dgrad_f);
+            g.cr_ticket = w.cr_ticket + 2 * (3 + l - 1);
             g.c.A = dre[l]; g.out_bf = dre[l - 1]; g.ldo = L.g.Cin;
             g.d_r = r[l - 1]; g.d_ld = L.g.Cin; g.d_act = ACT_SWISH;
             if (l > 1) { g.d_affine = w.aff_e[l - 2]; g.d_meanrstd = w.mr_e[l - 2]; g.d_red = w.red_e[l - 2]; }
@@ -1175,12 +1182,14 @@
         const ConvL& L = P.convT[l];
         if (name == "dec_convT" + std::to_string(l + 1)) {
             g = gemm_of(P, L.fwd, L.pk_fwd, 3, B, L.pk_fwd_f);
+            g.cr_ticket = w.cr_ticket + 2 * (6 + l);
             g.c.A = aq[l];
             g.out_bf = q[l + 1]; g.ldo = L.g.Cout; g.colstats = w.st_d[l];
             return true;
         }
         if (name == "dec_convT" + std::to_string(l + 1) + "_dgrad") {
             g = gemm_of(P, L.dgrad, L.pk_dgrad, 2, B, L.pk_dgrad_f);
+            g.cr_ticket = w.cr_ticket + 2 * (9 + l);
             g.c.A = dq[l + 1]; g.out_bf = dq[l]; g.ldo = L.g.Cin;
             g.d_r = q[l]; g.d_ld = L.g.Cin; g.d_act = ACT_SWISH;
             if (l > 0) { g.d_affine = w.aff_d[l - 1]; g.d_meanrstd = w.mr_d[l - 1]; g.d_red = w.red_d[l - 1]; }
```

Result: slower. 1660 ELBO-steps/s (-3.2%).
